# qq456cvb/CanonicalVoting

Hardware: AMD Instinct MI355X
Metric: scenes/sec (80k-pt synthetic scans) (higher is better)
Workload: dtype f32

## Files before the change

### canonicalvoting_amd/_lib.py

```python
import ctypes
import os
import threading

_HERE = os.path.dirname(os.path.abspath(__file__))
LIB_PATH = os.path.join(_HERE, "_C", "libcvhip.so")

c_float_p = ctypes.POINTER(ctypes.c_float)
c_int_p = ctypes.POINTER(ctypes.c_int)
c_i32_p = ctypes.POINTER(ctypes.c_int32)
c_i64_p = ctypes.POINTER(ctypes.c_int64)
vp = ctypes.c_void_p
ABI_VERSION = 6


class CvError(RuntimeError):
    pass


class DecodeParams(ctypes.Structure):
    _fields_ = [("thresh_high", ctypes.c_float), ("thresh_low", ctypes.c_float),
                ("valid_ratio", ctypes.c_float), ("elimination", ctypes.c_int),
                ("prob_thresh", ctypes.c_float), ("elim_hi_plus1", ctypes.c_int),
                ("max_iters", ctypes.c_int), ("err_thresh", ctypes.c_double)]

# ... 116 lines not shown
                ("d_points", vp), ("points_ld", ctypes.c_longlong), ("d_rgb", vp), ("d_owner", vp),
                ("d_minv", vp), ("d_model_scale", vp), ("d_model_cls", vp), ("n_models", ctypes.c_int),
                ("d_colour", vp), ("d_jitter", vp), ("n_clouds", ctypes.c_int),
                ("use_xyz", ctypes.c_int), ("recentre", ctypes.c_int),
                ("d_feats", vp), ("feats_ld", ctypes.c_longlong), ("d_xyz", vp), ("xyz_ld", ctypes.c_longlong),
                ("d_scale", vp), ("scale_ld", ctypes.c_longlong), ("d_cls", vp), ("cls_ld", ctypes.c_longlong)]


class SymLossDesc(ctypes.Structure):
    _fields_ = [("d_out", vp), ("n_rows", ctypes.c_longlong), ("ld", ctypes.c_longlong),
                ("d_rows", vp), ("d_pseg", vp), ("n_points", ctypes.c_longlong),
                ("d_seg_ptr", vp), ("d_pose_ptr", vp), ("d_tgt_ptr", vp), ("n_segments", ctypes.c_int), ("n_jobs", ctypes.c_int),
                ("d_targets", vp), ("n_targets", ctypes.c_longlong),
                ("d_urow", vp), ("d_uptr", vp), ("d_upoint", vp), ("n_urows", ctypes.c_int),
                ("w", ctypes.c_float * 3), ("xyz_factor", ctypes.c_float),
                ("d_loss", vp), ("d_pose_loss", vp), ("d_best", vp), ("d_seg_loss", vp),
                ("d_grad_loss", vp), ("d_grad", vp), ("grad_ld", ctypes.c_longlong),
                ("d_ws", vp), ("ws_bytes", ctypes.c_size_t)]


class SymRowsDesc(ctypes.Structure):
    _fields_ = [("d_coords4", vp), ("d_index", vp), ("d_inverse", vp), ("d_quant_counts", vp), ("m_points", ctypes.c_longlong),
                ("d_points", vp), ("points_ld", ctypes.c_longlong), ("d_rgb", vp), ("d_owner", vp),
                ("d_model_scale", vp), ("d_model_cls", vp), ("n_models", ctypes.c_int),
                ("d_colour", vp), ("d_jitter", vp), ("d_offsets", vp), ("n_clouds", ctypes.c_int),
                ("d_seg_vertex", vp), ("n_cand", ctypes.c_longlong),
                ("d_seg_vptr", vp), ("d_seg_pose_ptr", vp), ("n_seg_in", ctypes.c_int),
                ("d_minv", vp), ("n_jobs_in", ctypes.c_longlong), ("n_targets_in", ctypes.c_longlong),
                ("reference_indexing", ctypes.c_int), ("use_xyz", ctypes.c_int), ("recentre", ctypes.c_int),
                ("d_rows", vp), ("d_pseg", vp), ("d_seg_ptr", vp), ("d_pose_ptr", vp), ("d_tgt_ptr", vp), ("d_targets", vp),
                ("d_urow", vp), ("d_uptr", vp), ("d_upoint", vp),
                ("d_feats", vp), ("feats_ld", ctypes.c_longlong), ("d_scale", vp), ("scale_ld", ctypes.c_longlong),
                ("d_obj", vp), ("d_cls", vp), ("d_counts", vp), ("h_counts", vp),
                ("d_ws", vp), ("ws_bytes", ctypes.c_size_t)]


SYM_ROWS_COUNTS = ("P", "S", "J", "T", "U", "max_row", "N", "rejected")


class PointsFront(ctypes.Structure):
    _fields_ = [("d_raw_points", vp), ("m", ctypes.c_longlong), ("points_ld", ctypes.c_longlong), ("points_f64", ctypes.c_int),
                ("quantization_size", ctypes.c_double), ("d_raw_feats", vp), ("raw_feats_ld", ctypes.c_longlong),
                ("in_channels", ctypes.c_int), ("recentre_from", ctypes.c_int), ("d_raw_xyz", vp), ("d_raw_scale", vp),
                ("d_raw_prob", vp), ("d_raw_class", vp), ("d_coords4", vp), ("d_index", vp), ("d_inverse", vp)]


class PointsDesc(ctypes.Structure):
    _fields_ = [("front", PointsFront), ("scene", SceneDesc)]


class PointsSeparateDesc(ctypes.Structure):
    _fields_ = [("front", PointsFront), ("scene", SceneSeparateDesc)]


class PointsResult(ctypes.Structure):
    _fields_ = [("scene", SceneResult), ("n", ctypes.c_longlong), ("rejected", ctypes.c_int), ("host_us_front", ctypes.c_float),
                ("front_ws_bytes", ctypes.c_size_t), ("d_feats", vp), ("d_points", vp), ("d_xyz_in", vp), ("d_scale_in", vp),
                ("d_prob_in", vp), ("d_class_in", vp)]


class PointsSeparateResult(ctypes.Structure):
    _fields_ = [("scene", SceneSeparateResult), ("n", ctypes.c_longlong), ("rejected", ctypes.c_int),
                ("host_us_front", ctypes.c_float), ("front_ws_bytes", ctypes.c_size_t), ("d_feats", vp), ("d_points", vp),
                ("d_xyz_in", vp), ("d_scale_in", vp), ("d_prob_in", vp)]


SIGNATURES = {
    "cv_abi_version": (ctypes.c_int, []),
    "cv_last_error": (ctypes.c_char_p, []),
    "cv_hv_minmax_workspace_bytes": (ctypes.c_size_t, []),
    "cv_hv_minmax_f32": (ctypes.c_int, [vp, ctypes.c_int64, c_float_p, c_float_p, vp, ctypes.c_size_t, vp]),
    "cv_hv_minmax_async_f32": (ctypes.c_int, [vp, ctypes.c_int64, vp, vp, ctypes.c_size_t, vp]),
    "cv_hv_grid_dims_f32": (ctypes.c_int, [c_float_p, c_float_p, ctypes.c_float, c_int_p]),
    "cv_hv_forward_workspace_bytes": (ctypes.c_size_t, [ctypes.c_int64, ctypes.c_int, c_int_p, ctypes.c_int]),
    "cv_hv_forward_f32": (ctypes.c_int, [vp, vp, vp, vp, ctypes.c_int64, ctypes.c_float, ctypes.c_int,
                                         c_float_p, c_int_p, vp, vp, vp, vp, ctypes.c_size_t,
                                         ctypes.c_int, vp]),
    "cv_hv_forward_cat_workspace_bytes": (ctypes.c_size_t, [ctypes.c_int64, ctypes.c_int, c_int_p, ctypes.c_int, ctypes.c_int]),
    "cv_hv_forward_cat_f32": (ctypes.c_int, [vp, vp, vp, vp, ctypes.c_int64, ctypes.c_float, ctypes.c_int, c_float_p, c_int_p,
                                             ctypes.c_int, vp, vp, vp, vp, ctypes.c_size_t, ctypes.c_int, vp]),
    "cv_hv_forward_peaks_f32": (ctypes.c_int, [vp, vp, vp, vp, ctypes.c_int64, ctypes.c_float, ctypes.c_int,
                                               c_float_p, c_int_p, vp, vp, vp, vp, ctypes.c_size_t,
                                               ctypes.c_int, ctypes.c_float, vp]),
    "cv_hv_forward_peaks_cat_f32": (ctypes.c_int, [vp, vp, vp, vp, ctypes.c_int64, ctypes.c_float, ctypes.c_int, c_float_p, c_int_p,
                                                   ctypes.c_int, vp, vp, vp, vp, ctypes.c_size_t, ctypes.c_int, ctypes.c_float,
                                                   vp]),
    "cv_hv_set_kernel_events": (ctypes.c_int, [vp, vp]),
    "cv_hv_backward_f32": (ctypes.c_int, [vp, vp, vp, vp, vp, ctypes.c_int64, ctypes.c_float,
                                          ctypes.c_int, c_float_p, c_int_p, vp, vp, vp, vp]),
    "cv_hv_count_votes_f32": (ctypes.c_int, [vp, vp, vp, ctypes.c_int64, ctypes.c_float, ctypes.c_int,
                                             c_float_p, c_int_p, c_i64_p, vp, ctypes.c_size_t, vp]),
    "cv_decode_workspace_bytes": (ctypes.c_size_t, [c_int_p, ctypes.c_int64, ctypes.c_int]),
    "cv_decode_f32": (ctypes.c_int, [vp, vp, vp, c_int_p, c_float_p, ctypes.c_float, vp, vp, vp, vp,
                                     ctypes.c_int64, ctypes.POINTER(DecodeParams), ctypes.c_int, vp,
                                     ctypes.c_size_t, c_int_p, c_i64_p, c_i32_p, c_int_p, c_float_p,
                                     c_float_p, c_i32_p, c_int_p, vp]),
    "cv_decode_cat_workspace_bytes": (ctypes.c_size_t, [c_int_p, ctypes.c_int64, ctypes.c_int, ctypes.c_int]),
    "cv_decode_cat_f32": (ctypes.c_int, [vp, vp, vp, c_int_p, c_float_p, ctypes.c_float, vp, vp, vp, vp, ctypes.c_int64,
                                         ctypes.c_int, ctypes.POINTER(DecodeParams), ctypes.c_int, vp, ctypes.c_size_t, c_int_p,
                                         c_i64_p, c_i32_p, c_int_p, c_float_p, c_float_p, c_i32_p, c_int_p, vp]),
    "cv_detect_scene_separate_f32": (ctypes.c_int, [ctypes.POINTER(SceneSeparateDesc), ctypes.POINTER(SceneSeparateResult), vp]),
    "cv_sp_table_capacity": (ctypes.c_longlong, [ctypes.c_longlong]),
    "cv_sp_levels_workspace_bytes": (ctypes.c_size_t, [ctypes.c_longlong]),
    "cv_sp_build_levels": (ctypes.c_int, [ctypes.POINTER(vp), ctypes.POINTER(vp), ctypes.POINTER(vp),
                                          ctypes.c_longlong, ctypes.c_longlong, ctypes.c_int, vp,
                                          c_i32_p, vp, ctypes.c_size_t, vp]),
    "cv_sp_quantize_workspace_bytes": (ctypes.c_size_t, [ctypes.c_longlong]),
    "cv_sp_quantize_f32": (ctypes.c_int, [vp, ctypes.c_longlong, ctypes.c_longlong, ctypes.c_float, ctypes.c_int, c_i64_p,
                                          ctypes.c_int, vp, vp, vp, vp, c_i32_p, vp, ctypes.c_size_t, vp]),
    "cv_sp_quantize_f64": (ctypes.c_int, [vp, ctypes.c_longlong, ctypes.c_longlong, ctypes.c_double, ctypes.c_int, c_i64_p,
                                          ctypes.c_int, vp, vp, vp, vp, c_i32_p, vp, ctypes.c_size_t, vp]),
    "cv_sp_voxel_rows_f32": (ctypes.c_int, [vp, vp, ctypes.c_longlong, ctypes.c_float, vp, ctypes.POINTER(GatherJob), ctypes.c_int, vp]),
    "cv_sizeof_gather_job": (ctypes.c_size_t, []),
    "cv_sp_scan_rows_f32": (ctypes.c_int, [ctypes.POINTER(ScanRowsDesc), vp]),
    "cv_sizeof_scan_rows_desc": (ctypes.c_size_t, []),
    "cv_sym_loss_fwd_f32": (ctypes.c_int, [ctypes.POINTER(SymLossDesc), vp]),
    "cv_sym_loss_bwd_f32": (ctypes.c_int, [ctypes.POINTER(SymLossDesc), vp]),
    "cv_sym_loss_workspace_bytes": (ctypes.c_size_t, [ctypes.c_longlong, ctypes.c_int]),
    "cv_sym_loss_chunk_rows": (ctypes.c_int, []),
    "cv_sizeof_sym_loss_desc": (ctypes.c_size_t, []),
    "cv_sp_sym_rows_f32": (ctypes.c_int, [ctypes.POINTER(SymRowsDesc), vp]),
    "cv_sp_sym_rows_workspace_bytes": (ctypes.c_size_t, [ctypes.c_longlong, ctypes.c_longlong, ctypes.c_int, ctypes.c_int]),
    "cv_sp_sym_rows_block": (ctypes.c_int, []),
    "cv_sp_sym_rows_scan_span": (ctypes.c_longlong, []),
    "cv_sizeof_sym_rows_desc": (ctypes.c_size_t, []),
    "cv_sp_morton_keys": (ctypes.c_int, [vp, ctypes.c_longlong, vp, vp]),
    "cv_sp_sort_workspace_bytes": (ctypes.c_size_t, [ctypes.c_longlong]),
    "cv_sp_sort_rows": (ctypes.c_int, [vp, ctypes.c_longlong, vp, vp, vp, vp, ctypes.c_size_t, vp]),
    "cv_sp_pack_weights_stem_h2_f32": (ctypes.c_int, [vp, ctypes.c_int, ctypes.c_int, vp, ctypes.c_int, vp, vp]),
    "cv_sp_to_hl_f32": (ctypes.c_int, [vp, ctypes.c_longlong, ctypes.c_int, ctypes.c_int, vp, ctypes.c_int, vp, vp]),
    "cv_sp_from_hl_f32": (ctypes.c_int, [vp, ctypes.c_longlong, ctypes.c_int, ctypes.c_int, vp, ctypes.c_int, vp]),
    "cv_sp_kernel_map": (ctypes.c_int, [vp, ctypes.c_longlong, vp, vp, ctypes.c_longlong, ctypes.c_int,
                                        ctypes.c_int, vp, vp]),
    "cv_sp_up_map": (ctypes.c_int, [vp, ctypes.c_longlong, ctypes.c_longlong, vp, vp]),
    "cv_sp_conv_workspace_bytes": (ctypes.c_size_t, [ctypes.c_longlong, ctypes.c_int, ctypes.c_int]),
    "cv_sp_conv_f32": (ctypes.c_int, [ctypes.POINTER(ConvDesc), vp]),
    "cv_sp_set_split_target": (ctypes.c_int, [ctypes.c_int]),
    "cv_hv_set_part_records": (ctypes.c_int, [ctypes.c_int]),
    "cv_hv_set_part_records_thread": (ctypes.c_int, [ctypes.c_int]),
    "cv_sp_pack_weights_h2_batch_f32": (ctypes.c_int, [ctypes.POINTER(PackJob), ctypes.c_int, vp, vp]),
    "cv_sp_copy_unless_flag": (ctypes.c_int, [ctypes.POINTER(vp), ctypes.POINTER(vp), ctypes.POINTER(ctypes.c_longlong), ctypes.c_int, vp, vp]),
    "cv_sp_pack_weights_t_f32": (ctypes.c_int, [vp, ctypes.c_int, ctypes.c_int, ctypes.c_int, ctypes.c_int, ctypes.c_int, vp, vp]),
    "cv_sp_set_split_target_thread": (ctypes.c_int, [ctypes.c_int]),
    "cv_sp_set_ablation": (ctypes.c_int, [ctypes.c_int]),
    "cv_sp_set_option": (ctypes.c_int, [ctypes.c_char_p, ctypes.c_longlong, ctypes.POINTER(ctypes.c_longlong)]),
    "cv_sp_get_option": (ctypes.c_int, [ctypes.c_char_p, ctypes.POINTER(ctypes.c_longlong)]),
    "cv_sp_pack_weights_x6_f32": (ctypes.c_int, [vp, ctypes.c_int, ctypes.c_int, ctypes.c_int, vp, vp, vp]),
    "cv_sp_pack_weights_h2_f32": (ctypes.c_int, [vp, ctypes.c_int, ctypes.c_int, ctypes.c_int, vp, ctypes.c_int, vp, vp]),
    "cv_sp_pack_weights_bf16_f32": (ctypes.c_int, [vp, ctypes.c_int, ctypes.c_int, ctypes.c_int, vp, vp, vp]),
    "cv_sp_scene_maps_words": (ctypes.c_size_t, [c_i64_p, ctypes.c_longlong, ctypes.c_int, ctypes.c_int,
                                                 ctypes.c_longlong, ctypes.POINTER(SceneMaps)]),
    "cv_sp_scene_maps": (ctypes.c_int, [ctypes.POINTER(vp), ctypes.POINTER(vp), ctypes.POINTER(vp), ctypes.c_longlong,
                                        c_i64_p, vp, ctypes.c_longlong, ctypes.c_int,
                                        ctypes.c_int, ctypes.c_longlong, vp, ctypes.c_size_t, vp]),
    "cv_sp_scene_plan_words": (ctypes.c_size_t, [ctypes.c_longlong, ctypes.c_int, ctypes.c_int, ctypes.c_longlong]),
    "cv_sp_scene_plan": (ctypes.c_int, [vp, ctypes.c_longlong, vp, vp, ctypes.POINTER(vp), ctypes.POINTER(vp),
                                        ctypes.POINTER(vp), ctypes.c_longlong, vp, c_i32_p, ctypes.c_int, ctypes.c_int,
                                        ctypes.c_longlong, vp, ctypes.c_size_t, ctypes.POINTER(SceneMaps), vp,
                                        ctypes.c_size_t, vp, ctypes.c_size_t, vp]),
    "cv_sp_scene_plan_layout": (ctypes.c_int, [ctypes.c_longlong, ctypes.c_int, ctypes.c_int, ctypes.c_longlong,
                                               ctypes.POINTER(ScenePlanLayout)]),
    "cv_sp_scene_plan_slots": (ctypes.c_int, [ctypes.POINTER(ScenePlanLayout), ctypes.POINTER(SceneMaps), c_i64_p,
                                              ctypes.c_longlong, vp, ctypes.POINTER(vp), ctypes.POINTER(vp)]),
    "cv_sp_scene_conv_workspace_bytes": (ctypes.c_size_t, [c_i64_p, c_int_p, ctypes.c_int, ctypes.c_int]),
    "cv_net_arena_bytes": (ctypes.c_size_t, [ctypes.POINTER(NetBuf), ctypes.c_int, c_i64_p, ctypes.c_int]),
    "cv_net_run_f32": (ctypes.c_int, [ctypes.POINTER(NetOp), ctypes.c_int, ctypes.POINTER(NetBuf), ctypes.c_int,
# ... 111 lines not shown
```

### canonicalvoting_amd/csrc/cv_common.h

```cpp
#pragma once
#include <hip/hip_runtime.h>

#include <cstdarg>
#include <cstdint>
#include <cstdio>

#include "cv_hip.h"

void cv_set_error(const char* fmt, ...);

#define CV_HIP_CHECK(expr)                                                                  \
    do {                                                                                    \
        hipError_t e_ = (expr);                                                             \
        if (e_ != hipSuccess) {                                                             \
            cv_set_error("%s failed: %s (%s:%d)", #expr, hipGetErrorString(e_), __FILE__,   \
                         __LINE__);                                                         \
            return CV_EHIP;                                                                 \
        }                                                                                   \
    } while (0)

#define CV_LAUNCH_CHECK() CV_HIP_CHECK(hipGetLastError())

#define CV_REQUIRE(cond, code, ...)     \
    do {                                \
        if (!(cond)) {                  \
            cv_set_error(__VA_ARGS__);  \
            return (code);              \
        }                               \
    } while (0)

__host__ __device__ static inline size_t cv_align_up(size_t v, size_t a) { return (v + a - 1) / a * a; }

struct CvCarver {
    char* base;
    size_t off = 0;
    explicit CvCarver(void* p) : base(static_cast<char*>(p)) {}
    template <typename T>
    T* take(size_t count) {
        off = cv_align_up(off, 256);
        T* r = reinterpret_cast<T*>(base + off);
        off += count * sizeof(T);
        return r;
    }
};

struct CvMapJob {
    const int32_t* out_coords; long long n_out;
    const unsigned long long* keys; const int32_t* vals; long long cap;
    int k, ts;
    int32_t* nbr;
    const int32_t* compose;
    const unsigned* bitmap;
    const int32_t* bbox;
    int up;
    int32_t* nbr3;
    int32_t* mask_words;
};
constexpr int CV_MAX_MAP_JOBS = 12;
int cv_sp_kernel_maps_batch(const CvMapJob* jobs, int n_jobs, void* stream);
constexpr long long CV_BITMAP_WORDS = 1ll << 20;

int cv_sp_build_levels_zero(int32_t* const* d_coords, unsigned long long* const* d_keys, int32_t* const* d_vals,
                            long long n, long long cap, int num_levels, int32_t* d_counts, int32_t* h_counts, void* d_ws,
                            size_t ws_bytes, int32_t* d_zero, long long n_zero, int32_t* d_bbox, uint32_t* d_bits,
                            void* stream);

struct CvPermJob {
    const int32_t* nbr; long long n; int K, groups; int32_t* perm; int with_map;
    const int32_t* mask_words;
};
constexpr int CV_MAX_PERM_JOBS = 8;
int cv_hv_minmax_async_ex(const float* d_points, int64_t n, float* h_minmax6, void* d_ws, size_t ws_bytes, int32_t* d_zero_word,
                          int32_t* d_fill7f, void* stream);
struct DecodeCall {
    float* d_grid_obj; const float* d_grid_rot; const float* d_grid_scale;
    const int* dims; const float* h_corner3; float res;
    const float* d_points; const float* d_xyz; const float* d_prob; const int32_t* d_class; int64_t n;
    const cv_decode_params* params; int mutate_grid;
    void* d_ws; size_t ws_bytes;
    int* h_n_cand; int64_t* h_cand_idx; int32_t* h_verdict; int* h_n_boxes; float* h_boxes; float* h_scores; int32_t* h_classes;
    int* h_truncated;
    void* stream; void* ev_done;
};
int cv_decode_run(const DecodeCall& c, int num_cats, bool need_class);
int cv_sp_sort_rows_ex(const int32_t* d_coords, long long n, int32_t* d_sorted, int32_t* d_perm, int32_t* d_inv, void* d_ws,
                       size_t ws_bytes, bool single_batch, void* stream, bool bounds_prefilled);
int cv_sp_scene_plan_ex(const int32_t* d_input, long long n, int32_t* d_perm, int32_t* d_inv, int32_t* const* d_coords,
                        unsigned long long* const* d_keys, int32_t* const* d_vals, long long cap, int32_t* d_counts,
                        int32_t* h_counts, int stem_k, int mask_groups, long long masked_min_rows,
                        int32_t* d_arena, size_t arena_words, cv_scene_maps* offsets, void* d_sort_ws, size_t sort_ws_bytes,
                        void* d_levels_ws, size_t levels_ws_bytes, bool single_batch, void* stream,
                        bool bounds_prefilled);
int cv_sp_mask_perms_batch(const CvPermJob* jobs, int n_jobs, void* d_ws, size_t ws_bytes, void* stream,
                           bool pre_zeroed);

struct CvConvModels {
    int models;
    const cv_net_model_params* d_params;
    long long in_stride, in2_stride, res_stride, out_stride, ws_stride;
    int out_ext;
    float* ext_out[CV_MAX_CATEGORIES];
};
int cv_sp_conv_models_f32(const cv_conv_desc* d, const CvConvModels* mm, void* stream);
```

### canonicalvoting_amd/csrc/hv_decode.hip

```cpp
#include "cv_common.h"

#include <cmath>
#include <cstring>
#include <mutex>
#include <vector>

namespace {

constexpr int NCLS = 64;

struct Cand {
    long long idx;
    int c[3];
    int clo[3], chi[3];
    float cw[3];
    float cs, sn;
    float sc[3];
};

struct Stats {
    unsigned n_in, n_mask, pmax_bits;
    double err;
    unsigned hist[NCLS];
};
static_assert(offsetof(Stats, err) % 8 == 0, "64-bit atomic adds");
static_assert(sizeof(Stats) % 4 == 0, "a candidate's statistics are zeroed word by word");

struct Geo {
    int X, Y, Z;
    float corner[3];
    float res;
};

struct List {
    float* val;
    unsigned* xy;
    int* z;
    float* geo;
    int64_t cap;
};

__device__ __forceinline__ int cell_id(const Geo& geo, unsigned xy, int z) {
    return ((int)(xy & 0xffffu) * geo.Y + (int)(xy >> 16)) * geo.Z + z;
}

constexpr int CTR_WORDS = 16;
constexpr int CTR_LIST_N = 0;
constexpr int CTR_N_CAND = 4;

struct Ws {
    List L;
    unsigned* counters;
    Cand* cands;
    Stats* stats;
    __host__ __device__ unsigned* list_n() const { return counters + CTR_LIST_N; }
    __host__ __device__ int* n_cand() const { return reinterpret_cast<int*>(counters + CTR_N_CAND); }
};

struct CatStride { int64_t ws, n, cells; };
template <class T>
__device__ __forceinline__ void cat_shift(T*& p, int64_t bytes) {
    p = (T*)((char*)p + bytes);
}
__device__ __forceinline__ Ws cat(Ws w, int64_t stride, int k) {
    const int64_t o = (int64_t)k * stride;
    cat_shift(w.L.val, o); cat_shift(w.L.xy, o); cat_shift(w.L.z, o); cat_shift(w.L.geo, o);
    cat_shift(w.counters, o); cat_shift(w.cands, o); cat_shift(w.stats, o);
    return w;
}

__device__ __forceinline__ void lds_barrier() {
    asm volatile("s_waitcnt lgkmcnt(0)\n\ts_barrier" ::: "memory");
}

__device__ __forceinline__ int lanes_below(uint64_t mask) {
    return __builtin_amdgcn_mbcnt_hi((uint32_t)(mask >> 32),
                                     __builtin_amdgcn_mbcnt_lo((uint32_t)mask, 0));
}

__global__ __launch_bounds__(256) void dec_compact(const float* __restrict__ g_obj,
                                                   const float* __restrict__ g_rot,
                                                   const float* __restrict__ g_scale, Geo geo,
                                                   int64_t G, float thresh, Ws w, CatStride ks) {
    const int kc = blockIdx.y;
    g_obj = g_obj + kc * ks.cells; g_rot = g_rot + kc * 2 * ks.cells; g_scale = g_scale + kc * 3 * ks.cells;
    w = cat(w, ks.ws, kc);
    const List& L = w.L;
    unsigned* list_n = w.list_n();
    for (int64_t base = blockIdx.x * 256ll; base < G; base += (int64_t)gridDim.x * 256) {
        const int64_t i = base + threadIdx.x;
        float v = 0.f;
        bool hit = false;
        if (i < G) { v = g_obj[i]; hit = v >= thresh; }
        const uint64_t m = __ballot(hit);
        if (m == 0) continue;
        unsigned pos = 0;
        const int lane = threadIdx.x & 63;
        const int leader = __ffsll((unsigned long long)m) - 1;
        if (lane == leader) pos = atomicAdd(list_n, (unsigned)__popcll(m));
        pos = __shfl(pos, leader);
        if (hit) {
            const unsigned p = pos + lanes_below(m);
            const int id = (int)i;
            L.val[p] = v;
            const int z = id % geo.Z, y = (id / geo.Z) % geo.Y, x = id / (geo.Z * geo.Y);
            L.xy[p] = (unsigned)x | ((unsigned)y << 16);
            L.z[p] = z;
            const float r0 = g_rot[(int64_t)id * 2], r1 = g_rot[(int64_t)id * 2 + 1];
            const float rot = (float)atan2((double)r1, (double)r0);
            L.geo[0 * L.cap + p] = (float)cos((double)rot);
            L.geo[1 * L.cap + p] = (float)sin((double)rot);
            for (int k = 0; k < 3; ++k) L.geo[(2 + k) * L.cap + p] = g_scale[(int64_t)id * 3 + k];
        }
    }
}

__device__ __forceinline__ bool inv_coords(float d0, float d1, float d2, float c, float s,
                                           const float* sc, float& w0, float& w1, float& w2) {
    w0 = fmaf(d2, s, fmaf(d1, 0.f, d0 * c)) / sc[0];
    w1 = fmaf(d2, 0.f, fmaf(d1, 1.f, d0 * 0.f)) / sc[1];
    w2 = fmaf(d2, c, fmaf(d1, 0.f, d0 * (-s))) / sc[2];
    return -1 < w0 && w0 < 1 && -1 < w1 && w1 < 1 && -1 < w2 && w2 < 1;
}

__device__ __forceinline__ bool inside_box(float d0, float d1, float d2, float c, float s, const float* sc) {
    const float t0 = fmaf(d2, s, fmaf(d1, 0.f, d0 * c));
    const float t1 = fmaf(d2, 0.f, fmaf(d1, 1.f, d0 * 0.f));
    const float t2 = fmaf(d2, c, fmaf(d1, 0.f, d0 * (-s)));
    return fabsf(t0) < fabsf(sc[0]) && fabsf(t1) < fabsf(sc[1]) && fabsf(t2) < fabsf(sc[2]);
}

__device__ __forceinline__ void box_corners(float cs, float sn, const float* sc, float* bb) {
    constexpr float kRawX[8] = {1, 1, -1, -1, 1, 1, -1, -1};
    constexpr float kRawY[8] = {1, 1, 1, 1, -1, -1, -1, -1};
    constexpr float kRawZ[8] = {1, -1, -1, 1, 1, -1, -1, 1};
    const float m00 = cs * sc[0], m02 = (-sn) * sc[2], m11 = sc[1], m20 = sn * sc[0], m22 = cs * sc[2];
#pragma unroll
    for (int q = 0; q < 8; ++q) {
        bb[q * 3 + 0] = m00 * kRawX[q] + m02 * kRawZ[q];
        bb[q * 3 + 1] = m11 * kRawY[q];
        bb[q * 3 + 2] = m20 * kRawX[q] + m22 * kRawZ[q];
    }
}

struct Best {
    float v;
    int id, pos;
    int q;
};

__device__ __forceinline__ void take_better(Best& b, float v, int id, int pos, int q) {
    if (v > b.v || (v == b.v && id < b.id)) { b.v = v; b.id = id; b.pos = pos; b.q = q; }
}

constexpr int GREEDY_T = 512;
constexpr int GREEDY_CAP = 4096;

template <int CTRL>
__device__ __forceinline__ int dpp_mov(int x) {
    return __builtin_amdgcn_update_dpp(x, x, CTRL, 0xf, 0xf, false);
}
__device__ __forceinline__ float wave_max_f32(float x) {
    x = fmaxf(x, __int_as_float(dpp_mov<0xB1>(__float_as_int(x))));
    x = fmaxf(x, __int_as_float(dpp_mov<0x4E>(__float_as_int(x))));
    x = fmaxf(x, __int_as_float(dpp_mov<0x124>(__float_as_int(x))));
    x = fmaxf(x, __int_as_float(dpp_mov<0x128>(__float_as_int(x))));
    const int xi = __float_as_int(x);
    const float a = __int_as_float(__builtin_amdgcn_readlane(xi, 0)), b = __int_as_float(__builtin_amdgcn_readlane(xi, 16)),
                c = __int_as_float(__builtin_amdgcn_readlane(xi, 32)), d = __int_as_float(__builtin_amdgcn_readlane(xi, 48));
    return fmaxf(fmaxf(a, b), fmaxf(c, d));
}
__device__ __forceinline__ int wave_min_i32(int x) {
    x = min(x, dpp_mov<0xB1>(x));
    x = min(x, dpp_mov<0x4E>(x));
    x = min(x, dpp_mov<0x124>(x));
    x = min(x, dpp_mov<0x128>(x));
    return min(min(__builtin_amdgcn_readlane(x, 0), __builtin_amdgcn_readlane(x, 16)),
               min(__builtin_amdgcn_readlane(x, 32), __builtin_amdgcn_readlane(x, 48)));
}

template <int W, class Also>
__device__ __forceinline__ Best best_of_workgroup(float (&s_val)[2][W], int (&s_idx)[2][W], int (&s_pos)[2][W], int it, float bv,
                                                  int bid, int bpos, Also&& also) {
    const int wave = threadIdx.x >> 6, par = it & 1;
    const float wv = wave_max_f32(bv);
    const int wid = wave_min_i32(bv == wv ? bid : 0x7fffffff);
    if (bv == wv && bid == wid) {
        s_val[par][wave] = bv; s_idx[par][wave] = bid; s_pos[par][wave] = bpos;
        also(par, wave);
    }
    lds_barrier();
    Best w{s_val[par][0], s_idx[par][0], s_pos[par][0], 0};
#pragma unroll
    for (int q = 1; q < W; ++q) take_better(w, s_val[par][q], s_idx[par][q], s_pos[par][q], q);
    return w;
// ... 472 lines not shown
    const int nx = cd.chi[0] - cd.clo[0] + 1, ny = cd.chi[1] - cd.clo[1] + 1,
              nz = cd.chi[2] - cd.clo[2] + 1;
    for (int64_t t = threadIdx.x; t < (int64_t)nx * ny * nz; t += 256) {
        const int z = cd.clo[2] + (int)(t % nz), y = cd.clo[1] + (int)((t / nz) % ny),
                  x = cd.clo[0] + (int)(t / ((int64_t)nz * ny));
        float w0, w1, w2;
        if (inv_coords((float)(x - cd.c[0]) * geo.res, (float)(y - cd.c[1]) * geo.res,
                       (float)(z - cd.c[2]) * geo.res, cd.cs, cd.sn, cd.sc, w0, w1, w2))
            g_obj[((int64_t)x * geo.Y + y) * geo.Z + z] = 0.f;
    }
}

__global__ __launch_bounds__(64) void dec_zero_counters(Ws w, int64_t ks_ws) {
    w = cat(w, ks_ws, blockIdx.y);
    if (threadIdx.x < CTR_WORDS) w.counters[threadIdx.x] = 0u;
}

struct WsLayout {
    size_t off_val, off_xy, off_z, off_geo, off_counters, off_cands, off_stats, total;
    int64_t cells;
    WsLayout(int64_t G, int M) : cells(G) {
        size_t o = 0;
        off_val = o; o = cv_align_up(o + sizeof(float) * G, 256);
        off_xy = o; o = cv_align_up(o + sizeof(unsigned) * G, 256);
        off_z = o; o = cv_align_up(o + sizeof(int) * G, 256);
        off_geo = o; o = cv_align_up(o + sizeof(float) * 5 * G, 256);
        off_counters = o; o = cv_align_up(o + sizeof(unsigned) * CTR_WORDS, 256);
        off_cands = o; o = cv_align_up(o + sizeof(Cand) * M, 256);
        off_stats = o; o = cv_align_up(o + sizeof(Stats) * M, 256);
        o = cv_align_up(o + ResultLayout(M).total, 256);
        total = o;
    }
    Ws at(char* ws) const {
        Ws w;
        w.L.val = reinterpret_cast<float*>(ws + off_val);
        w.L.xy = reinterpret_cast<unsigned*>(ws + off_xy);
        w.L.z = reinterpret_cast<int*>(ws + off_z);
        w.L.geo = reinterpret_cast<float*>(ws + off_geo);
        w.L.cap = cells;
        w.counters = reinterpret_cast<unsigned*>(ws + off_counters);
        w.cands = reinterpret_cast<Cand*>(ws + off_cands);
        w.stats = reinterpret_cast<Stats*>(ws + off_stats);
        return w;
    }
};

struct PinnedPool {
    std::mutex mu;
    std::vector<std::pair<char*, size_t>> free_list;
    std::pair<char*, size_t> take(size_t bytes) {
        {
            std::lock_guard<std::mutex> g(mu);
            for (size_t i = 0; i < free_list.size(); ++i)
                if (free_list[i].second >= bytes) {
                    const std::pair<char*, size_t> b = free_list[i];
                    free_list.erase(free_list.begin() + i);
                    return b;
                }
        }
        void* p = nullptr;
        if (hipHostMalloc(&p, bytes, hipHostMallocMapped) != hipSuccess) return {nullptr, 0};
        return {static_cast<char*>(p), bytes};
    }
    void give(std::pair<char*, size_t> b) {
        std::lock_guard<std::mutex> g(mu);
        if (free_list.size() < 64) free_list.push_back(b);
        else (void)hipHostFree(b.first);
    }
};
PinnedPool g_pinned;

struct PinnedLease {
    const std::pair<char*, size_t> buf;
    explicit PinnedLease(size_t bytes) : buf(g_pinned.take(bytes)) {}
    ~PinnedLease() { if (buf.first) g_pinned.give(buf); }
    PinnedLease(const PinnedLease&) = delete;
    PinnedLease& operator=(const PinnedLease&) = delete;
};

}

int cv_decode_run(const DecodeCall& c, int K, bool need_class) {
    CV_REQUIRE(K >= 1 && K <= CV_MAX_CATEGORIES, CV_EINVAL, "num_cats out of range (%d, 1..%d)", K, CV_MAX_CATEGORIES);
    CV_REQUIRE(c.d_grid_obj && c.d_grid_rot && c.d_grid_scale && c.dims && c.h_corner3 && c.d_points && c.d_xyz && c.d_prob &&
                   (c.d_class || !need_class) && c.params && c.d_ws && c.h_n_cand && c.h_cand_idx && c.h_verdict && c.h_n_boxes &&
                   c.h_boxes && c.h_scores && c.h_classes,
               CV_EINVAL, "null pointer argument");
    const int* dims = c.dims;
    const cv_decode_params* params = c.params;
    const int64_t n = c.n;
    hipStream_t st = static_cast<hipStream_t>(c.stream);
    CV_REQUIRE(n > 0, CV_EINVAL, "n must be positive");
    CV_REQUIRE(c.res > 0.f, CV_EINVAL, "res must be positive");
    CV_REQUIRE(dims[0] > 0 && dims[1] > 0 && dims[2] > 0, CV_EINVAL, "bad grid dims");
    CV_REQUIRE(dims[0] < 65536 && dims[1] < 65536 && dims[2] < 65536, CV_EINVAL, "grid dims must be below 65536");
    const int64_t G = (int64_t)dims[0] * dims[1] * dims[2];
    CV_REQUIRE(G < (1ll << 31), CV_EINVAL, "grid too large");
    const int M = params->max_iters;
    CV_REQUIRE(M > 0 && M <= 65536, CV_EINVAL, "max_iters out of range");
    CV_REQUIRE(params->elimination >= 0, CV_EINVAL, "elimination must be >= 0");
    CV_REQUIRE(params->thresh_high > 0.f, CV_EINVAL, "thresh_high must be positive");
    const WsLayout W(G, M);
    const size_t need = (size_t)K * W.total;
    CV_REQUIRE(c.ws_bytes >= need, CV_ENOMEM, "workspace too small (%zu < %zu)", c.ws_bytes, need);
    const Ws w = W.at(static_cast<char*>(c.d_ws));
    const ResultLayout RL(M);
    const PinnedLease lease((size_t)K * RL.total);
    char* host = lease.buf.first;
    CV_REQUIRE(host != nullptr, CV_ENOMEM, "pinned host buffer of %zu bytes", (size_t)K * RL.total);
    const CatStride ks{K > 1 ? (int64_t)W.total : 0, n, G};

    if (K == 1) CV_HIP_CHECK(hipMemsetAsync(w.counters, 0, sizeof(unsigned) * CTR_WORDS, st));
    else {
        dec_zero_counters<<<dim3(1, K), 64, 0, st>>>(w, ks.ws);
        CV_LAUNCH_CHECK();
    }
    Geo geo{dims[0], dims[1], dims[2], {c.h_corner3[0], c.h_corner3[1], c.h_corner3[2]}, c.res};
    const int cblocks = (int)std::min<int64_t>((G + 255) / 256, 2048);
    dec_compact<<<dim3(cblocks, K), 256, 0, st>>>(c.d_grid_obj, c.d_grid_rot, c.d_grid_scale, geo, G, params->thresh_high, w, ks);
    CV_LAUNCH_CHECK();
    static const long long big_cells = getenv("CV_DEC_BIG_CELLS") ? atoll(getenv("CV_DEC_BIG_CELLS")) : (4ll << 20);
    if (G > big_cells) dec_greedy_dispatch_big<<<dim3(1, K), GREEDY_T_BIG, 0, st>>>(geo, *params, w, ks.ws);
    else dec_greedy_dispatch<<<dim3(1, K), GREEDY_T, 0, st>>>(geo, *params, w, ks.ws);
    CV_LAUNCH_CHECK();
    const dim3 bgrid((unsigned)((n + 255) / 256), (unsigned)std::min((M + 7) / 8, 8), (unsigned)K);
    dec_backproject<<<bgrid, 256, 0, st>>>(c.d_points, c.d_xyz, c.d_prob, c.d_class, n, params->prob_thresh, w, ks);
    CV_LAUNCH_CHECK();
    dec_finalize<<<dim3(1, K), 256, 0, st>>>(w, *params, host, M, ks.ws, (int64_t)RL.total);
    CV_LAUNCH_CHECK();
    if (c.mutate_grid) {
        dec_apply<<<dim3(M, K), 256, 0, st>>>(c.d_grid_obj, geo, *params, w, ks);
        CV_LAUNCH_CHECK();
    }
    if (c.ev_done) CV_HIP_CHECK(hipEventRecord(static_cast<hipEvent_t>(c.ev_done), st));
    CV_HIP_CHECK(hipStreamSynchronize(st));
    for (int k = 0; k < K; ++k) {
        const char* hk = host + (size_t)k * RL.total;
        const int* hdr = reinterpret_cast<const int*>(hk);
        const int nc = hdr[0], nb = hdr[1];
        CV_REQUIRE(nc >= 0 && nc <= M && nb >= 0 && nb <= nc, CV_ERANGE, "corrupt decode result");
        c.h_n_cand[k] = nc;
        c.h_n_boxes[k] = nb;
        if (c.h_truncated) c.h_truncated[k] = hdr[2];
        std::memcpy(c.h_cand_idx + (size_t)k * M, hk + RL.off_cand, sizeof(int64_t) * nc);
        std::memcpy(c.h_verdict + (size_t)k * M, hk + RL.off_verdict, sizeof(int32_t) * nc);
        std::memcpy(c.h_boxes + (size_t)k * M * 24, hk + RL.off_boxes, sizeof(float) * 24 * nb);
        std::memcpy(c.h_scores + (size_t)k * M, hk + RL.off_scores, sizeof(float) * nb);
        std::memcpy(c.h_classes + (size_t)k * M, hk + RL.off_classes, sizeof(int32_t) * nb);
    }
    return CV_OK;
}

extern "C" {

size_t cv_decode_workspace_bytes(const int dims[3], int64_t n, int max_iters) {
    if (!dims || max_iters <= 0) return 0;
    (void)n;
    return WsLayout((int64_t)dims[0] * dims[1] * dims[2], max_iters).total;
}

size_t cv_decode_cat_workspace_bytes(const int dims[3], int64_t n, int max_iters, int num_cats) {
    if (num_cats < 1 || num_cats > CV_MAX_CATEGORIES) return 0;
    return (size_t)num_cats * cv_decode_workspace_bytes(dims, n, max_iters);
}

int cv_decode_f32(float* d_grid_obj, const float* d_grid_rot, const float* d_grid_scale,
                  const int dims[3], const float h_corner3[3], float res, const float* d_points,
                  const float* d_xyz, const float* d_prob, const int32_t* d_class, int64_t n,
                  const cv_decode_params* params, int mutate_grid, void* d_ws, size_t ws_bytes,
                  int* h_n_cand, int64_t* h_cand_idx, int32_t* h_verdict, int* h_n_boxes,
                  float* h_boxes, float* h_scores, int32_t* h_classes, int* h_truncated, void* stream) {
    const DecodeCall c{d_grid_obj, d_grid_rot, d_grid_scale, dims, h_corner3, res, d_points, d_xyz, d_prob, d_class, n, params,
                       mutate_grid, d_ws, ws_bytes, h_n_cand, h_cand_idx, h_verdict, h_n_boxes, h_boxes, h_scores, h_classes,
                       h_truncated, stream, nullptr};
    return cv_decode_run(c, 1, true);
}

int cv_decode_cat_f32(float* d_grid_obj, const float* d_grid_rot, const float* d_grid_scale, const int dims[3],
                      const float h_corner3[3], float res, const float* d_points, const float* d_xyz, const float* d_prob,
                      const int32_t* d_class, int64_t n, int num_cats, const cv_decode_params* params, int mutate_grid, void* d_ws,
                      size_t ws_bytes, int* h_n_cand, int64_t* h_cand_idx, int32_t* h_verdict, int* h_n_boxes, float* h_boxes,
                      float* h_scores, int32_t* h_classes, int* h_truncated, void* stream) {
    const DecodeCall c{d_grid_obj, d_grid_rot, d_grid_scale, dims, h_corner3, res, d_points, d_xyz, d_prob, d_class, n, params,
                       mutate_grid, d_ws, ws_bytes, h_n_cand, h_cand_idx, h_verdict, h_n_boxes, h_boxes, h_scores, h_classes,
                       h_truncated, stream, nullptr};
    return cv_decode_run(c, num_cats, false);
}

}
```

### canonicalvoting_amd/csrc/hv_vote.hip

```cpp
#include "cv_common.h"

#include <atomic>
#include <algorithm>
#include <cmath>
#include <cstddef>
#include <mutex>
#include <type_traits>
#include <unordered_map>
#include <vector>

namespace {

struct F3 { float x, y, z; };
struct I3 { int x, y, z; };

std::mutex g_tab_mu;
std::unordered_map<uint64_t, float2*> g_tabs;

int get_rot_table(int num_rots, const float2** out) {
    int dev = 0;
    CV_HIP_CHECK(hipGetDevice(&dev));
    const uint64_t key = (uint64_t(uint32_t(dev)) << 32) | uint32_t(num_rots);
    std::lock_guard<std::mutex> lk(g_tab_mu);
    auto it = g_tabs.find(key);
// ... 132 lines not shown

constexpr int TX = 16, TZ = 32, TCELLS = TX * TZ;
constexpr int TW = 8;
constexpr int LQ = TW * 64;
constexpr int CULL_BATCH = 4;
static_assert(CULL_BATCH >= 1 && CULL_BATCH <= 8, "one carry bit and one record index per sub-chunk and lane");
constexpr int VQ = 128;
constexpr int MAX_R_TILES = 256;
static_assert(MAX_R_TILES <= TW * 64, "the rotation table is staged by one load per lane");
constexpr int LIST_CHUNK = 16;
static_assert(64 % LIST_CHUNK == 0, "a wave takes 64 / LIST_CHUNK list chunks per hand-out, one entry per lane");
static_assert(LQ <= 512, "the list entry of a queued vote has 9 bits");
static_assert(MAX_R_TILES <= 256, "the rotation of a queued vote has 8 bits");
static_assert(TX + 1 < 64 && TZ + 1 < 64, "lx + 1 and lz + 1 of a queued vote have 6 bits each");
static_assert(TZ == 32, "acc_idx splits a cell index by >> 5 and & 31");

constexpr int LIST_CHUNK_RECORDS = 1024;
constexpr int PREP_MAX_Y = 4096;
constexpr int PREP_THREADS = 1024;

struct CatStride { int64_t ws, n, cells; };
template <class T>
__device__ __forceinline__ T* cat_ws(T* p, int64_t bytes) {
    return (T*)((const char*)p + (int64_t)blockIdx.y * bytes);
}
template <class T>
__device__ __forceinline__ T* cat_el(T* p, int64_t elems) {
    return p + (int64_t)blockIdx.y * elems;
}

__global__ __launch_bounds__(PREP_THREADS) void hv_prep_count(
    const float* __restrict__ pts, const float* __restrict__ xyz, const float* __restrict__ scl,
    int64_t n, float res, float corner_y, int Y, int* __restrict__ fy_out, int* __restrict__ ycount, CatStride ks) {
    __shared__ int lh[PREP_MAX_Y];
    xyz = cat_el(xyz, 3 * ks.n); scl = cat_el(scl, 3 * ks.n);
    fy_out = cat_ws(fy_out, ks.ws); ycount = cat_ws(ycount, ks.ws);
    const bool use_lds = Y <= PREP_MAX_Y;
    if (use_lds) {
        for (int i = threadIdx.x; i < Y; i += PREP_THREADS) lh[i] = 0;
        __syncthreads();
    }
    const int64_t c = blockIdx.x * (int64_t)PREP_THREADS + threadIdx.x;
    if (c < n) {
        const float cy = xyz[c * 3 + 1] * scl[c * 3 + 1];
        const float gy = grid_pos(pts[c * 3 + 1], -cy, corner_y, res);
        int fy = -1;
        if (gy >= 0 && gy < (float)(Y - 1)) fy = (int)gy;
        fy_out[c] = fy;
        if (fy >= 0) atomicAdd(use_lds ? &lh[fy] : &ycount[fy], 1);
    }
    if (use_lds) {
        __syncthreads();
        for (int i = threadIdx.x; i < Y; i += PREP_THREADS)
            if (lh[i]) atomicAdd(&ycount[i], lh[i]);
    }
}

constexpr int PART_RECORDS = 4096;
constexpr int MAX_PARTS = 8;

template <class V, class E>
__device__ __forceinline__ int wave_excl_scan(int Y, V value, E emit) {
    const int lane = threadIdx.x & 63;
    int carry = 0;
    for (int base = 0; base < Y; base += 64) {
        const int i = base + lane;
        const int v = i < Y ? value(i) : 0;
        int incl = v;
#pragma unroll
        for (int off = 1; off < 64; off <<= 1) {
            const int t = __shfl_up(incl, off);
            if (lane >= off) incl += t;
        }
        if (i < Y) emit(i, carry + incl - v, v);
        carry += __shfl(incl, 63);
    }
    return carry;
}
__global__ __launch_bounds__(256) void hv_prep_scan(const int* __restrict__ ycount, int Y,
                                                    int* __restrict__ ystart,
                                                    int* __restrict__ cursor,
                                                    int* __restrict__ part_start, int4* __restrict__ q_info, int max_q,
                                                    int* __restrict__ chunk_start, int* __restrict__ bin_of_chunk,
                                                    int part_records, int64_t ks_ws) {
    ycount = cat_ws(ycount, ks_ws); ystart = cat_ws(ystart, ks_ws); cursor = cat_ws(cursor, ks_ws);
    part_start = cat_ws(part_start, ks_ws); q_info = cat_ws(q_info, ks_ws);
    chunk_start = cat_ws(chunk_start, ks_ws); bin_of_chunk = cat_ws(bin_of_chunk, ks_ws);
    const int wave = threadIdx.x >> 6, lane = threadIdx.x & 63;
    if (wave == 0) {
        const int total = wave_excl_scan(Y, [&](int i) { return ycount[i]; },
                                         [&](int i, int excl, int) { ystart[i] = excl; cursor[i] = excl; });
        if (lane == 0) ystart[Y] = total;
    } else if (wave == 1) {
        const int total = wave_excl_scan(Y,
            [&](int i) {
                const int n2 = (i >= 1 ? ycount[i - 1] : 0) + (i <= Y - 2 ? ycount[i] : 0);
                return min(max((n2 + part_records - 1) / part_records, 1), MAX_PARTS);
            },
            [&](int i, int excl, int v) {
                part_start[i] = excl;
                for (int p2 = 0; p2 < v; ++p2) q_info[excl + p2] = make_int4(i, p2, v, excl);
            });
        for (int q = total + lane; q < max_q; q += 64) q_info[q] = make_int4(0, 0, -1, 0);
        if (lane == 0) part_start[Y] = total;
    } else if (wave == 2) {
        const int total = wave_excl_scan(Y, [&](int i) { return (ycount[i] + LIST_CHUNK_RECORDS - 1) / LIST_CHUNK_RECORDS; },
                                         [&](int i, int excl, int v) {
                                             chunk_start[i] = excl;
                                             for (int p2 = 0; p2 < v; ++p2) bin_of_chunk[excl + p2] = i;
                                         });
        if (lane == 0) chunk_start[Y] = total;
    }
}

constexpr int REC_F = 13;

__global__ __launch_bounds__(PREP_THREADS) void hv_prep_scatter(
    const float* __restrict__ pts, const float* __restrict__ xyz, const float* __restrict__ scl,
    const float* __restrict__ obj, const int* __restrict__ fy_in, int64_t n, int Y, float res,
    F3 corner, int* __restrict__ cursor, float* __restrict__ rec, int64_t rec_stride, CatStride ks) {
    __shared__ int lh[PREP_MAX_Y];
    xyz = cat_el(xyz, 3 * ks.n); scl = cat_el(scl, 3 * ks.n); obj = cat_el(obj, ks.n);
    fy_in = cat_ws(fy_in, ks.ws); cursor = cat_ws(cursor, ks.ws); rec = cat_ws(rec, ks.ws);
    const bool use_lds = Y <= PREP_MAX_Y;
    const int64_t c = blockIdx.x * (int64_t)PREP_THREADS + threadIdx.x;
    const int fy = c < n ? fy_in[c] : -1;
    int pos = -1;
    if (!use_lds) {
        if (fy >= 0) pos = atomicAdd(&cursor[fy], 1);
    } else {
        for (int i = threadIdx.x; i < Y; i += PREP_THREADS) lh[i] = 0;
        __syncthreads();
        int rank = 0;
        if (fy >= 0) rank = atomicAdd(&lh[fy], 1);
        __syncthreads();
        for (int i = threadIdx.x; i < Y; i += PREP_THREADS)
            if (lh[i]) lh[i] = atomicAdd(&cursor[i], lh[i]);
        __syncthreads();
        if (fy >= 0) pos = lh[fy] + rank;
    }
    if (pos < 0) return;
    const float px = pts[c * 3 + 0], py = pts[c * 3 + 1], pz = pts[c * 3 + 2];
    const float s0 = scl[c * 3 + 0], s1 = scl[c * 3 + 1], s2 = scl[c * 3 + 2];
    const float cx = xyz[c * 3 + 0] * s0, cy = xyz[c * 3 + 1] * s1, cz = xyz[c * 3 + 2] * s2;
    const float gy = grid_pos(py, -cy, corner.y, res);
    float* r = rec + pos;
    r[0 * rec_stride] = px;
    r[1 * rec_stride] = pz;
    r[2 * rec_stride] = cx;
    r[3 * rec_stride] = cz;
    r[4 * rec_stride] = gy - floorf(gy);
    r[5 * rec_stride] = obj[c];
    r[6 * rec_stride] = s0;
    r[7 * rec_stride] = s1;
    r[8 * rec_stride] = s2;
    r[9 * rec_stride] = (px - corner.x) / res;
    r[10 * rec_stride] = (pz - corner.z) / res;
    r[11 * rec_stride] = sqrtf(cx * cx + cz * cz) / res;
    r[12 * rec_stride] = atan2f(cz, cx) + 3.14159265f;
}


constexpr int LIST_MAX_TILES = 4096;
struct RingArc { bool keep; int a_start, a_len; };
__device__ __forceinline__ bool ring_touches(float ux, float uz, float r, float xlo, float xhi, float zlo, float zhi,
                                             float& dxn, float& dzn) {
    const float slack = 0.05f;
    dxn = fmaxf(0.f, fmaxf(xlo - ux, ux - xhi));
    dzn = fmaxf(0.f, fmaxf(zlo - uz, uz - zhi));
    const float dxf = fmaxf(fabsf(ux - xlo), fabsf(ux - xhi));
    const float dzf = fmaxf(fabsf(uz - zlo), fabsf(uz - zhi));
    const float dmin = sqrtf(dxn * dxn + dzn * dzn), dmax = sqrtf(dxf * dxf + dzf * dzf);
    const float tol = slack + 1e-5f * (r + fabsf(ux) + fabsf(uz));
    return (r >= dmin - tol) && (r <= dmax + tol);
}
__device__ __forceinline__ void ring_arc(float ux, float uz, float a0, int R, float xlo, float xhi, float zlo, float zhi,
                                         float dxn, float dzn, int& a_start, int& a_len) {
    a_start = 0;
    a_len = R;
    if (dxn + dzn > 0.5f) {
        const float b0 = atan2f(0.5f * (zlo + zhi) - uz, 0.5f * (xlo + xhi) - ux);
        float lo = 0.f, hi = 0.f;
#pragma unroll
        for (int k = 0; k < 4; ++k) {
            float d = atan2f(((k & 2) ? zhi : zlo) - uz, ((k & 1) ? xhi : xlo) - ux) - b0;
            d -= 6.28318531f * rintf(d * 0.159154943f);
            lo = fminf(lo, d);
            hi = fmaxf(hi, d);
        }
        const float inv_step = (float)R * 0.159154943f;
        float first = (b0 + lo - a0) * inv_step - 2.f;
        const int len = (int)((hi - lo) * inv_step) + 6;
        first -= (float)R * floorf(first / (float)R);
        a_start = min(max((int)first, 0), R - 1);
// ... 228 lines not shown
        rx = sh.vq_rx[wave][slot]; rz = sh.vq_rz[wave][slot];
        const int e = rec & 511, rot = (rec >> 9) & 255;
        lx = (int)((rec >> 17) & 63) - 1; lz = (int)((rec >> 23) & 63) - 1;
        wy = sh.pq[4][e]; ob = sh.pq[5][e];
        if constexpr (MODE != VOTE_OBJ) {
            s0 = sh.pq[6][e]; s1 = sh.pq[7][e]; s2 = sh.pq[8][e];
            cs = sh.tab[rot];
        }
    }
    const bool small = fabsf(ob) * fmaxf(1.f, fmaxf(fabsf(s0), fmaxf(fabsf(s1), fabsf(s2)))) < 16384.f;
    if (__all(small)) {
        if (active) drain_vote<true, MODE>(sh, lx, lz, rx, rz, wy, ob, s0, s1, s2, cs, box);
    } else {
        if (active) drain_vote<false, MODE>(sh, lx, lz, rx, rz, wy, ob, s0, s1, s2, cs, box);
    }
}

__device__ __forceinline__ void wave_sync_lds() {
    __builtin_amdgcn_fence(__ATOMIC_RELEASE, "wavefront");
    __builtin_amdgcn_wave_barrier();
    __builtin_amdgcn_fence(__ATOMIC_ACQUIRE, "wavefront");
}

__device__ __forceinline__ float arc_atan2(float y, float x) {
    const float ax = fabsf(x), ay = fabsf(y);
    const float a = fminf(ax, ay) * __builtin_amdgcn_rcpf(fmaxf(fmaxf(ax, ay), 1e-30f));
    const float q = a * a;
    float r = ((-0.0464964749f * q + 0.15931422f) * q - 0.327622764f) * q * a + a;
    r = ay > ax ? 1.57079637f - r : r;
    r = x < 0.f ? 3.14159274f - r : r;
    return y < 0.f ? -r : r;
}

__device__ __forceinline__ void edge_arc(float ux, float uz, float r, float a0, int R, float xlo, float xhi, float zlo,
                                         float zhi, int& a_start, int& a_len) {
    if (!(r >= 2.f)) return;
    const float slack = 0.05f, half_pi = 1.57079637f, two_pi = 6.28318531f;
    const float d4[4] = {xhi - ux, zhi - uz, ux - xlo, uz - zlo};
    const float inv_r = 1.f / r;
    float h[4];
#pragma unroll
    for (int k = 0; k < 4; ++k) {
        const float t = (d4[k] + slack) * inv_r;
        const float hk = arc_atan2(sqrtf(fmaxf(1.f - t * t, 0.f)), t) - 0.01f;
        h[k] = (t < 1.f && hk > 0.f) ? hk : -1.f;
    }
    float best = 0.f, best_end = 0.f;
#pragma unroll
    for (int k = 0; k < 4; ++k) {
        float lo = -h[k], hi = h[k];
        bool ok = h[k] > 0.f;
        if (ok && hi - lo > best) { best = hi - lo; best_end = (float)k * half_pi + hi; }
#pragma unroll
        for (int j = 1; j < 4; ++j) {
            const float hp = h[(k + j - 1) & 3], hn = h[(k + j) & 3];
            ok = ok && hn > 0.f && hp + hn >= half_pi;
            if (ok) {
                lo = fminf(lo, (float)j * half_pi - hn);
                hi = fmaxf(hi, (float)j * half_pi + hn);
                if (hi - lo > best) { best = hi - lo; best_end = (float)k * half_pi + hi; }
            }
        }
    }
    const float inside = fmaxf(two_pi - best, 0.f);
    const float inv_step = (float)R * 0.159154943f;
    const int len = (int)(inside * inv_step) + 6;
    if (len < a_len) {
        float first = (best_end - a0) * inv_step - 2.f;
        first -= (float)R * floorf(first / (float)R);
        a_start = min(max((int)first, 0), R - 1);
        a_len = len;
    }
}

template <bool QUEUE, int MODE>
__device__ __forceinline__ void hv_tile_item(
    int y, int tile, int part, int nparts, int slot0, int slot_stride,
    int R, float res, F3 corner, I3 dims,
    const int* __restrict__ ystart, const float* __restrict__ rec,
    int64_t rec_stride, int tiles_x, int tiles_z, unsigned long long* __restrict__ partials,
    int* __restrict__ arrivals, float* __restrict__ g_obj, float* __restrict__ g_rot,
    float* __restrict__ g_scale, const int* __restrict__ list_ctl, const int* __restrict__ list_start, const int* __restrict__ list_cnt,
    const int2* __restrict__ entries, int list_mode ,
    int4* __restrict__ hot, float thresh, int4* __restrict__ hot_items, const float2* __restrict__ tab) {
    constexpr int NCH = vote_channels(MODE);
    __shared__ TileSharedT<MODE> sh;
    __shared__ int last_flag;
    __shared__ int hot_lds[MODE == VOTE_OBJ ? 4 : 1];
    const int X = dims.x, Y = dims.y, Z = dims.z;
    const int ntiles = tiles_x * tiles_z;
    const int x0 = (tile / tiles_z) * TX, z0 = (tile % tiles_z) * TZ;
    const int lane = threadIdx.x & 63, wave = threadIdx.x >> 6;
    HotBox box{0, TX - 1, 0, TZ - 1};
    if (MODE == VOTE_PEAKS) {
        const int4 h = hot[y * ntiles + tile];
        box = HotBox{h.x, h.y, h.z, h.w};
        if (box.x0 > box.x1) return;
    }
    if (nparts == 0) {
        const int nx0 = min(TX, X - x0), nz0 = min(TZ, Z - z0);
        for (int i = threadIdx.x; i < TCELLS; i += TW * 64) {
            const int lx = i / TZ, lz = i % TZ;
            if (lx < nx0 && lz < nz0) {
                const int64_t cell = ((int64_t)(x0 + lx) * Y + y) * Z + z0 + lz;
                if (MODE != VOTE_PEAKS) g_obj[cell] = 0.f;
                if (MODE != VOTE_OBJ) {
                    reinterpret_cast<float2*>(g_rot)[cell] = make_float2(0.f, 0.f);
                    g_scale[cell * 3 + 0] = 0.f; g_scale[cell * 3 + 1] = 0.f; g_scale[cell * 3 + 2] = 0.f;
                }
            }
        }
        if (MODE == VOTE_OBJ && threadIdx.x == 0) {
            hot[y * ntiles + tile] = 0.f >= thresh ? make_int4(0, nx0 - 1, 0, nz0 - 1) : make_int4(TX, -1, TZ, -1);
            if (0.f >= thresh) hot_items[atomicAdd(&arrivals[Y * ntiles], 1)] = make_int4(y, tile, 0, slot0);
        }
        return;
    }
    const bool use_list = QUEUE && list_mode == 2 && list_ctl[1] == 0;
    int lbeg[2] = {0, 0}, llen[2] = {0, 0};
    if (use_list) {
#pragma unroll
        for (int k = 0; k < 2; ++k) {
            const int s = y - 1 + k;
            if (s >= 0 && s <= Y - 2) {
                lbeg[k] = list_start[(int64_t)s * ntiles + tile];
                llen[k] = list_cnt[(int64_t)s * ntiles + tile];
            }
        }
    }

    int bin_beg[2], bin_end[2];
#pragma unroll
    for (int k = 0; k < 2; ++k) {
        const int s = y - 1 + k;
        const bool valid = s >= 0 && s <= Y - 2;
        bin_beg[k] = !valid ? 0 : (use_list ? lbeg[k] : ystart[s]);
        bin_end[k] = !valid ? 0 : (use_list ? lbeg[k] + llen[k] : ystart[s + 1]);
    }
    const float2 tab_mine = (int)threadIdx.x < R ? tab[threadIdx.x] : make_float2(0.f, 0.f);
    for (int i = threadIdx.x; i < TileSharedT<MODE>::ACC_WORDS; i += TW * 64) sh.acc[i] = 0ull;
    if ((int)threadIdx.x < R) sh.tab[threadIdx.x] = tab_mine;
    if (threadIdx.x < 2) sh.next_chunk[threadIdx.x] = 0;
    if (threadIdx.x == 2) { sh.list_len = 0; sh.more = 0; }
    if (MODE == VOTE_OBJ && threadIdx.x >= 4 && threadIdx.x < 8)
        hot_lds[threadIdx.x - 4] = (threadIdx.x & 1) ? -1 : (threadIdx.x == 4 ? TX : TZ);
    __syncthreads();

    const float slack = 0.05f;
    const float xlo = MODE == VOTE_PEAKS ? (float)(x0 + box.x0 - 1) : (float)(x0 - 1),
                xhi = MODE == VOTE_PEAKS ? (float)(x0 + box.x1 + 1) : (float)(x0 + TX),
                zlo = MODE == VOTE_PEAKS ? (float)(z0 + box.z0 - 1) : (float)(z0 - 1),
                zhi = MODE == VOTE_PEAKS ? (float)(z0 + box.z1 + 1) : (float)(z0 + TZ);
    int vq_len = 0;

    const int per = use_list ? LIST_CHUNK : 64;
    int sb = 0;
    int c_mask = 0, c_idx[CULL_BATCH], c_arc = 0, c_k = 0;
#pragma unroll
    for (int j = 0; j < CULL_BATCH; ++j) c_idx[j] = 0;
    auto append = [&](int mask, const int (&idx)[CULL_BATCH], int arc, int k) -> int {
        int tot = 0, before[CULL_BATCH];
#pragma unroll
        for (int j = 0; j < CULL_BATCH; ++j) {
            const uint64_t m = __ballot((mask >> j) & 1);
            before[j] = tot + lanes_below(m);
            tot += __popcll(m);
        }
        if (tot == 0) return 0;
        int p0 = 0;
        if (lane == 0) p0 = atomicAdd(&sh.list_len, tot);
        p0 = __builtin_amdgcn_readfirstlane(p0);
#pragma unroll
        for (int j = 0; j < CULL_BATCH; ++j) {
            const int pos = p0 + before[j];
            if (((mask >> j) & 1) && pos < LQ) {
                sh.arc_start[pos] = idx[j] | (int)((unsigned)k << 31);
                if (use_list) sh.arc_cum[pos] = arc;
                mask &= ~(1 << j);
            }
        }
        return mask;
    };

    for (;;) {
        bool more = false;
        if (__ballot(c_mask != 0) != 0) {
            c_mask = append(c_mask, c_idx, c_arc, c_k);
            more = __ballot(c_mask != 0) != 0;
        }
// ... 151 lines not shown
            float rx = 0, rz = 0;
            if (it0 < it1) {
                if (it0 == e_end) {
                    ++e;
                    e_end = sh.arc_cum[e];
                    rot = sh.arc_start[e];
                    epx = sh.pq[0][e]; epz = sh.pq[1][e];
                    ecx = sh.pq[2][e]; ecz = sh.pq[3][e];
                }
                const float2 cs = sh.tab[rot];
                const float ox = (-cs.x) * ecx + cs.y * ecz;
                const float oz = (-cs.y) * ecx - cs.x * ecz;
                const float gx = grid_pos(epx, ox, corner.x, res);
                const float gz = grid_pos(epz, oz, corner.z, res);
                if (gx >= 0 && gz >= 0 && gx < (float)(X - 1) && gz < (float)(Z - 1)) {
                    const int lx = (int)gx - x0, lz = (int)gz - z0;
                    if (MODE == VOTE_PEAKS ? (lx >= box.x0 - 1 && lx <= box.x1 && lz >= box.z0 - 1 && lz <= box.z1)
                                           : (lx >= -1 && lx < TX && lz >= -1 && lz < TZ)) {
                        isvote = true;
                        rx = gx - floorf(gx);
                        rz = gz - floorf(gz);
                        vrec = (uint32_t)e | ((uint32_t)rot << 9) | ((uint32_t)(lx + 1) << 17) |
                               ((uint32_t)(lz + 1) << 23);
                    }
                }
                if (++rot == R) rot = 0;
            }
            const uint64_t mv = __ballot(isvote);
            if (isvote) {
                const int q = vq_len + lanes_below(mv);
                sh.vq_rec[wave][q] = vrec;
                sh.vq_rx[wave][q] = rx;
                sh.vq_rz[wave][q] = rz;
            }
            vq_len += __popcll(mv);
            wave_sync_lds();
            if (vq_len >= 64) {
                vq_len -= 64;
                drain64<MODE>(sh, wave, vq_len + lane, true, box);
            }
        }
        if (vq_len > 0) {
            drain64<MODE>(sh, wave, lane, lane < vq_len, box);
            vq_len = 0;
        }
        wave_sync_lds();
        if (!again) break;
        __syncthreads();
    }
    __syncthreads();

    if (nparts > 1) {
        unsigned long long* mine = partials + ((int64_t)slot0 + (int64_t)part * slot_stride) * (6 * TCELLS);
        for (int i = threadIdx.x; i < NCH * TCELLS; i += TW * 64) mine[i] = sh.acc[acc_idx(i / TCELLS, i % TCELLS)];
        asm volatile("s_waitcnt vmcnt(0)" ::: "memory");
        __syncthreads();
        if (threadIdx.x == 0) {
            __builtin_amdgcn_fence(__ATOMIC_RELEASE, "agent");
            asm volatile("s_waitcnt vmcnt(0)" ::: "memory");
            const int old = __hip_atomic_fetch_add(&arrivals[y * ntiles + tile], 1, __ATOMIC_RELAXED,
                                                   __HIP_MEMORY_SCOPE_AGENT);
            last_flag = old == nparts - 1;
            if (last_flag) __builtin_amdgcn_fence(__ATOMIC_ACQUIRE, "agent");
            if (MODE == VOTE_OBJ && last_flag)
                __hip_atomic_store(&arrivals[y * ntiles + tile], 0, __ATOMIC_RELAXED, __HIP_MEMORY_SCOPE_AGENT);
        }
        __syncthreads();
        if (!last_flag) return;
        const unsigned long long* base = partials + (int64_t)slot0 * (6 * TCELLS);
        for (int i = threadIdx.x; i < NCH * TCELLS; i += TW * 64) {
            unsigned long long sum = 0ull;
            for (int p2 = 0; p2 < nparts; ++p2) sum += base[(int64_t)p2 * slot_stride * (6 * TCELLS) + i];
            sh.acc[acc_idx(i / TCELLS, i % TCELLS)] = sum;
        }
        __syncthreads();
    }

    const int nx = min(TX, X - x0), nz = min(TZ, Z - z0);
    if constexpr (MODE == VOTE_OBJ) {
        for (int i = threadIdx.x; i < TCELLS; i += TW * 64) {
            const int lx = i / TZ, lz = i % TZ;
            if (lx < nx && lz < nz) {
                const float v = (float)fx_value(sh.acc[acc_idx(0, i)]);
                g_obj[((int64_t)(x0 + lx) * Y + y) * Z + z0 + lz] = v;
                if (v >= thresh) {
                    atomicMin(&hot_lds[0], lx); atomicMax(&hot_lds[1], lx);
                    atomicMin(&hot_lds[2], lz); atomicMax(&hot_lds[3], lz);
                }
            }
        }
        __syncthreads();
        if (threadIdx.x == 0) {
            hot[y * ntiles + tile] = make_int4(hot_lds[0], hot_lds[1], hot_lds[2], hot_lds[3]);
            if (hot_lds[0] <= hot_lds[1]) {
                const int at = atomicAdd(&arrivals[Y * ntiles], nparts);
                for (int p2 = 0; p2 < nparts; ++p2) hot_items[at + p2] = make_int4(y, tile, p2 | (nparts << 8), slot0);
            }
        }
    } else if constexpr (MODE == VOTE_PEAKS) {
        for (int i = threadIdx.x; i < TCELLS; i += TW * 64) {
            const int lx = i / TZ, lz = i % TZ;
            if (lx < box.x0 || lx > box.x1 || lz < box.z0 || lz > box.z1) continue;
            const int64_t cell = ((int64_t)(x0 + lx) * Y + y) * Z + z0 + lz;
            const float v = g_obj[cell];
            if (!(v >= thresh)) continue;
            const double d = (double)v + 1e-7;
#pragma unroll
            for (int j = 0; j < 2; ++j) g_rot[cell * 2 + j] = (float)((double)(float)fx_value(sh.acc[acc_idx(j, i)]) / d);
#pragma unroll
            for (int j = 0; j < 3; ++j) g_scale[cell * 3 + j] = (float)((double)(float)fx_value(sh.acc[acc_idx(2 + j, i)]) / d);
        }
    } else {
        for (int i = threadIdx.x; i < TCELLS; i += TW * 64) {
            const int lx = i / TZ, lz = i % TZ;
            if (lx < nx && lz < nz)
                g_obj[((int64_t)(x0 + lx) * Y + y) * Z + z0 + lz] = (float)fx_value(sh.acc[acc_idx(0, i)]);
        }
        for (int i = threadIdx.x; i < TCELLS * 2; i += TW * 64) {
            const int cell = i >> 1, j = i & 1;
            const int lx = cell / TZ, lz = cell % TZ;
            if (lx < nx && lz < nz) {
                const double d = (double)(float)fx_value(sh.acc[acc_idx(0, cell)]) + 1e-7;
                g_rot[(((int64_t)(x0 + lx) * Y + y) * Z + z0 + lz) * 2 + j] =
                    (float)((double)(float)fx_value(sh.acc[acc_idx(1 + j, cell)]) / d);
            }
        }
        for (int i = threadIdx.x; i < TCELLS * 3; i += TW * 64) {
            const int cell = i / 3, j = i - cell * 3;
            const int lx = cell / TZ, lz = cell % TZ;
            if (lx < nx && lz < nz) {
                const double d = (double)(float)fx_value(sh.acc[acc_idx(0, cell)]) + 1e-7;
                g_scale[(((int64_t)(x0 + lx) * Y + y) * Z + z0 + lz) * 3 + j] =
                    (float)((double)(float)fx_value(sh.acc[acc_idx(3 + j, cell)]) / d);
            }
        }
    }
}

template <bool QUEUE, int MODE>
__global__ __launch_bounds__(TW * 64) void hv_fwd_tiles(
    int R, float res, F3 corner, I3 dims, const float2* __restrict__ tab,
    const int* __restrict__ ystart, const int4* __restrict__ items, const float* __restrict__ rec,
    int64_t rec_stride, int tiles_x, int tiles_z, unsigned long long* __restrict__ partials,
    int* __restrict__ arrivals, float* __restrict__ g_obj, float* __restrict__ g_rot,
    float* __restrict__ g_scale, const int* __restrict__ list_ctl, const int* __restrict__ list_start, const int* __restrict__ list_cnt,
    const int2* __restrict__ entries, int list_mode ,
    const int4* __restrict__ q_info, CatStride ks, int4* __restrict__ hot, float thresh, int4* __restrict__ hot_items) {
    ystart = cat_ws(ystart, ks.ws); items = cat_ws(items, ks.ws); rec = cat_ws(rec, ks.ws);
    partials = cat_ws(partials, ks.ws); arrivals = cat_ws(arrivals, ks.ws); list_ctl = cat_ws(list_ctl, ks.ws);
    list_start = cat_ws(list_start, ks.ws); list_cnt = cat_ws(list_cnt, ks.ws); entries = cat_ws(entries, ks.ws);
    q_info = cat_ws(q_info, ks.ws);
    g_obj = cat_el(g_obj, ks.cells); g_rot = cat_el(g_rot, 2 * ks.cells); g_scale = cat_el(g_scale, 3 * ks.cells);
    if (MODE != VOTE_FULL) { hot = cat_ws(hot, ks.ws); hot_items = cat_ws(hot_items, ks.ws); }
    const int ntiles = tiles_x * tiles_z;
#define CV_TILE_ITEM_ARGS R, res, corner, dims, ystart, rec, rec_stride, tiles_x, tiles_z, partials, arrivals, g_obj, g_rot, g_scale, \
                          list_ctl, list_start, list_cnt, entries, list_mode, hot, thresh, hot_items
    if (MODE == VOTE_PEAKS) {
        const int count = arrivals[dims.y * ntiles];
        if ((int)blockIdx.x >= count) return;
        for (int i = blockIdx.x; i < count; i += gridDim.x) {
            const int4 item = hot_items[i];
            hv_tile_item<QUEUE, MODE>(item.x, item.y, item.z & 0xff, item.z >> 8, item.w, QUEUE ? 1 : ntiles, CV_TILE_ITEM_ARGS, tab);
            __syncthreads();
        }
        return;
    }
    int y, tile, part, nparts, slot0, slot_stride;
    if (QUEUE) {
        if ((int)blockIdx.x >= list_ctl[2]) return;
        const int4 item = items[blockIdx.x];
        y = item.x; tile = item.y; part = item.z & 0xff; nparts = item.z >> 8; slot0 = item.w; slot_stride = 1;
    } else {
        tile = blockIdx.x % ntiles;
        const int4 qi = q_info[blockIdx.x / ntiles];
        if (qi.z < 0) return;
        y = qi.x; part = qi.y; nparts = qi.z;
        slot0 = qi.w * ntiles + tile; slot_stride = ntiles;
    }
    hv_tile_item<QUEUE, MODE>(y, tile, part, nparts, slot0, slot_stride, CV_TILE_ITEM_ARGS, tab);
#undef CV_TILE_ITEM_ARGS
}

__global__ __launch_bounds__(256) void hv_bwd(
    const float* __restrict__ grad, const float* __restrict__ pts, const float* __restrict__ xyz,
    const float* __restrict__ scl, const float* __restrict__ obj, int64_t n, int R, float res,
    F3 corner, I3 dims, const float2* __restrict__ tab, float* __restrict__ d_xyz,
    float* __restrict__ d_scl, float* __restrict__ d_obj) {
    const int lane = threadIdx.x & 63;
    const int64_t c = blockIdx.x * 4ll + (threadIdx.x >> 6);
    if (c >= n) return;
    const int Y = dims.y, Z = dims.z;
    const float s0 = scl[c * 3 + 0], s1 = scl[c * 3 + 1], s2 = scl[c * 3 + 2];
    const float x0 = xyz[c * 3 + 0], x1 = xyz[c * 3 + 1], x2 = xyz[c * 3 + 2];
    const float cx = x0 * s0, cy = x1 * s1, cz = x2 * s2;
    const float px = pts[c * 3 + 0], py = pts[c * 3 + 1], pz = pts[c * 3 + 2];
    const float ob = obj[c];
    float a_obj = 0, a_x0 = 0, a_x1 = 0, a_x2 = 0, a_s0 = 0, a_s1 = 0, a_s2 = 0;
    for (int i = lane; i < R; i += 64) {
        const float2 cs = tab[i];
        const float ox = (-cs.x) * cx + cs.y * cz;
        const float oy = -cy;
        const float oz = (-cs.y) * cx - cs.x * cz;
        const float gx = grid_pos(px, ox, corner.x, res);
        const float gy = grid_pos(py, oy, corner.y, res);
        const float gz = grid_pos(pz, oz, corner.z, res);
        if (gx < 0 || gy < 0 || gz < 0 || gx >= (float)(dims.x - 1) || gy >= (float)(dims.y - 1) ||
            gz >= (float)(dims.z - 1))
            continue;
        const int fx = (int)gx, fy = (int)gy, fz = (int)gz;
        const float rx = gx - floorf(gx), ry = gy - floorf(gy), rz = gz - floorf(gz);
        const float w0x = 1.f - rx, w0y = 1.f - ry, w0z = 1.f - rz, w1x = rx, w1y = ry, w1z = rz;
        const int64_t b = ((int64_t)fx * Y + fy) * Z + fz;
        const int64_t sx = (int64_t)Y * Z, sy = Z;
        const float lll = grad[b], llh = grad[b + 1], lhl = grad[b + sy], lhh = grad[b + sy + 1];
        const float hll = grad[b + sx], hlh = grad[b + sx + 1], hhl = grad[b + sx + sy],
                    hhh = grad[b + sx + sy + 1];
        float dob = lll * w0x * w0y * w0z;
        dob += llh * w0x * w0y * w1z;
        dob += lhl * w0x * w1y * w0z;
        dob += lhh * w0x * w1y * w1z;
        dob += hll * w1x * w0y * w0z;
        dob += hlh * w1x * w0y * w1z;
        dob += hhl * w1x * w1y * w0z;
        dob += hhh * w1x * w1y * w1z;
        a_obj += dob;
        float dx = -lll * w0y * w0z;
        dx = dx - llh * w0y * w1z; dx = dx - lhl * w1y * w0z; dx = dx - lhh * w1y * w1z;
        dx = dx + hll * w0y * w0z; dx = dx + hlh * w0y * w1z; dx = dx + hhl * w1y * w0z;
        dx = dx + hhh * w1y * w1z;
        float dy = -lll * w0x * w0z;
        dy = dy - llh * w0x * w1z; dy = dy + lhl * w0x * w0z; dy = dy + lhh * w0x * w1z;
        dy = dy - hll * w1x * w0z; dy = dy - hlh * w1x * w1z; dy = dy + hhl * w1x * w0z;
        dy = dy + hhh * w1x * w1z;
        float dz = -lll * w0x * w0y;
        dz = dz + llh * w0x * w0y; dz = dz - lhl * w0x * w1y; dz = dz + lhh * w0x * w1y;
        dz = dz - hll * w1x * w0y; dz = dz + hlh * w1x * w0y; dz = dz - hhl * w1x * w1y;
        dz = dz + hhh * w1x * w1y;
        dx *= ob; dy *= ob; dz *= ob;
        const float dcx = (-cs.x) * dx - cs.y * dz;
// ... 152 lines not shown
    const int rc = cv_hv_minmax_async_ex(d_points, n, h, d_ws, ws_bytes, nullptr, nullptr, stream);
    if (rc) return rc;
    CV_HIP_CHECK(hipStreamSynchronize(static_cast<hipStream_t>(stream)));
    for (int k = 0; k < 3; ++k) { h_min3[k] = h[k]; h_max3[k] = h[3 + k]; }
    return CV_OK;
}

int cv_hv_minmax_async_f32(const float* d_points, int64_t n, float* h_minmax6, void* d_ws, size_t ws_bytes,
                           void* stream) {
    return cv_hv_minmax_async_ex(d_points, n, h_minmax6, d_ws, ws_bytes, nullptr, nullptr, stream);
}

}

int cv_hv_minmax_async_ex(const float* d_points, int64_t n, float* h_minmax6, void* d_ws, size_t ws_bytes, int32_t* d_zero_word,
                          int32_t* d_fill7f, void* stream) {
    CV_REQUIRE(d_points && h_minmax6 && d_ws, CV_EINVAL, "null pointer argument");
    CV_REQUIRE(n > 0, CV_EINVAL, "n must be positive (got %lld)", (long long)n);
    CV_REQUIRE(ws_bytes >= cv_hv_minmax_workspace_bytes(), CV_ENOMEM, "workspace too small");
    hipStream_t st = static_cast<hipStream_t>(stream);
    CvCarver cv(d_ws);
    float* part = cv.take<float>(6 * MM_BLOCKS);
    float* out = cv.take<float>(6);
    const int blocks = (int)std::min<int64_t>(MM_BLOCKS, (n + 255) / 256);
    minmax_partial<<<blocks, 256, 0, st>>>(d_points, n, part);
    CV_LAUNCH_CHECK();
    minmax_final<<<1, 256, 0, st>>>(part, blocks, out, d_zero_word, d_fill7f);
    CV_LAUNCH_CHECK();
    CV_HIP_CHECK(hipMemcpyAsync(h_minmax6, out, 6 * sizeof(float), hipMemcpyDeviceToHost, st));
    return CV_OK;
}

extern "C" {

int cv_hv_grid_dims_f32(const float h_min3[3], const float h_max3[3], float res, int dims_out[3]) {
    CV_REQUIRE(h_min3 && h_max3 && dims_out, CV_EINVAL, "null pointer argument");
    CV_REQUIRE(res > 0.f, CV_EINVAL, "res must be positive");
    for (int k = 0; k < 3; ++k) {
        volatile float d = h_max3[k] - h_min3[k];
        volatile float q = d / res;
        dims_out[k] = (int)q + 1;
    }
    return CV_OK;
}

size_t cv_hv_forward_workspace_bytes(int64_t n, int num_rots, const int dims[3], int algo) {
    if (!dims || n <= 0 || !algo_ok(algo)) return 0;
    if (pick_algo(algo, n, num_rots) == 1) return 256;
    return tiles_layout(n, num_rots, dims, nullptr).bytes;
}

static thread_local hipEvent_t t_ev_start = nullptr, t_ev_stop = nullptr;

static std::atomic<long long> g_part_records{getenv("CV_HV_PART_RECORDS") ? std::max<long long>(PART_RECORDS, atoll(getenv("CV_HV_PART_RECORDS")))
                                                                          : (long long)PART_RECORDS};

static thread_local long long t_part_records = 0;

int cv_hv_set_part_records(int records) {
    const long long v = records <= 0 ? (long long)PART_RECORDS : std::max<long long>(PART_RECORDS, records);
    return (int)g_part_records.exchange(v, std::memory_order_relaxed);
}

int cv_hv_set_part_records_thread(int records) {
    const int before = (int)t_part_records;
    t_part_records = records <= 0 ? 0 : std::max<long long>(PART_RECORDS, records);
    return before;
}

int cv_hv_set_kernel_events(void* ev_start, void* ev_stop) {
    t_ev_start = static_cast<hipEvent_t>(ev_start);
    t_ev_stop = static_cast<hipEvent_t>(ev_stop);
    return CV_OK;
}

size_t cv_hv_forward_cat_workspace_bytes(int64_t n, int num_rots, const int dims[3], int algo, int num_cats) {
    if (num_cats < 1 || num_cats > CV_MAX_CATEGORIES) return 0;
    return (size_t)num_cats * cv_hv_forward_workspace_bytes(n, num_rots, dims, algo);
}

static int hv_forward_cats(const float* d_points, const float* d_xyz, const float* d_scale, const float* d_obj, int64_t n,
                           float res, int num_rots, const float h_corner3[3], const int dims[3], float* d_grid_obj,
                           float* d_grid_rot, float* d_grid_scale, void* d_ws, size_t ws_bytes, int algo, int K,
                           hipStream_t st, bool peaks = false, float thresh = 0.f) {
    int rc = CV_OK;
    const float2* tab = nullptr;
    rc = get_rot_table(num_rots, &tab);
    if (rc) return rc;
    const F3 corner{h_corner3[0], h_corner3[1], h_corner3[2]};
    const I3 d3{dims[0], dims[1], dims[2]};
    const int64_t cells = (int64_t)dims[0] * dims[1] * dims[2];
    const int a = pick_algo(algo, n, num_rots);
    if (a == 2) CV_REQUIRE(num_rots <= MAX_R_TILES, CV_EINVAL, "tiles algorithm needs num_rots <= %d", MAX_R_TILES);
    if (a == 1) {
        for (int k = 0; k < K; ++k) {
            float* g_obj = d_grid_obj + (int64_t)k * cells;
            float* g_rot = d_grid_rot + (int64_t)k * cells * 2;
            float* g_scale = d_grid_scale + (int64_t)k * cells * 3;
            CV_HIP_CHECK(hipMemsetAsync(g_obj, 0, sizeof(float) * cells, st));
            CV_HIP_CHECK(hipMemsetAsync(g_rot, 0, sizeof(float) * cells * 2, st));
            CV_HIP_CHECK(hipMemsetAsync(g_scale, 0, sizeof(float) * cells * 3, st));
            const int64_t total = n * num_rots;
            hv_fwd_direct<<<(unsigned)((total + 255) / 256), 256, 0, st>>>(
                d_points, d_xyz + (int64_t)k * n * 3, d_scale + (int64_t)k * n * 3, d_obj + (int64_t)k * n, n, num_rots, res,
                corner, d3, tab, g_obj, g_rot, g_scale);
            CV_LAUNCH_CHECK();
            hv_normalise<<<(unsigned)((cells + 255) / 256), 256, 0, st>>>(g_obj, g_rot, g_scale, cells);
            CV_LAUNCH_CHECK();
        }
        return CV_OK;
    }
    const int Y = dims[1];
    const TilesLayout L = tiles_layout(n, num_rots, dims, d_ws);
    CV_REQUIRE(d_ws && ws_bytes >= (size_t)K * L.bytes, CV_ENOMEM, "workspace too small for the tiles algorithm");
    const CatStride ks{K > 1 ? (int64_t)L.bytes : 0, n, cells};
    const int tiles_x = L.tiles_x, tiles_z = L.tiles_z, ntiles = L.ntiles;
    const bool queue = L.queue;
    const int list_mode = queue ? 2 : 1;
    if (K == 1) CV_HIP_CHECK(hipMemsetAsync(L.zero_from, 0, L.zero_bytes, st));
    else {
        hv_zero_cat<<<dim3((unsigned)std::min<size_t>((L.zero_bytes / 4 + 255) / 256, 1024), K), 256, 0, st>>>(L.zero_from,
                                                                                                          L.zero_bytes / 4, ks.ws);
        CV_LAUNCH_CHECK();
    }
    const unsigned prep_wgs = (unsigned)((n + PREP_THREADS - 1) / PREP_THREADS);
    hv_prep_count<<<dim3(prep_wgs, K), PREP_THREADS, 0, st>>>(d_points, d_xyz, d_scale, n, res, corner.y, Y, L.fy, L.ycount, ks);
    CV_LAUNCH_CHECK();
    hv_prep_scan<<<dim3(1, K), 256, 0, st>>>(L.ycount, Y, L.ystart, L.cursor, L.part_start, L.q_info, (int)L.max_q, L.chunk_start,
                                             L.bin_of_chunk,
                                             (int)(t_part_records > 0 ? t_part_records : g_part_records.load(std::memory_order_relaxed)),
                                             ks.ws);
    CV_LAUNCH_CHECK();
    hv_prep_scatter<<<dim3(prep_wgs, K), PREP_THREADS, 0, st>>>(d_points, d_xyz, d_scale, d_obj, L.fy, n, Y, res, corner, L.cursor,
                                                                 L.rec, n, ks);
    CV_LAUNCH_CHECK();
    if (queue) {
        hv_list_pass<false><<<dim3((unsigned)L.max_chunks, K), 1024, 0, st>>>(L.ystart, L.chunk_start, L.bin_of_chunk, Y, L.rec, n,
                                                                               num_rots, tiles_x, tiles_z, L.list_ctl, L.list_cnt,
                                                                               L.list_start, L.chunk_off, L.entries, L.tile_w, 1, ks.ws);
        CV_LAUNCH_CHECK();
        hv_build_queue<<<dim3(1, K), 1024, 0, st>>>(L.tile_w, Y, ntiles, (int)L.max_items, (int)L.max_slots, L.list_ctl, L.items,
                                                    ks.ws);
        CV_LAUNCH_CHECK();
        hv_list_scan<<<dim3(1, K), 1024, 0, st>>>(L.list_cnt, Y, ntiles, L.list_cap, L.list_ctl, L.list_start, ks.ws);
        CV_LAUNCH_CHECK();
        hv_list_pass<true><<<dim3((unsigned)L.max_chunks, K), 1024, 0, st>>>(L.ystart, L.chunk_start, L.bin_of_chunk, Y, L.rec, n,
                                                                              num_rots, tiles_x, tiles_z, L.list_ctl, L.list_cnt,
                                                                              L.list_start, L.chunk_off, L.entries, L.tile_w, 1, ks.ws);
        CV_LAUNCH_CHECK();
    }
    const int64_t wgs = queue ? L.max_items : L.max_q * ntiles;
    CV_REQUIRE(wgs < (1ll << 31), CV_EINVAL, "grid too large");
#define CV_TILES_ARGS num_rots, res, corner, d3, tab, L.ystart, L.items, L.rec, n, tiles_x, tiles_z, L.partials, L.arrivals, d_grid_obj, \
                      d_grid_rot, d_grid_scale, L.list_ctl, L.list_start, L.list_cnt, L.entries, list_mode, L.q_info, ks, L.hot, thresh, L.hot_items
#define CV_TILES_LAUNCH(MODE, WGS)                                                                           \
    do {                                                                                                      \
        if (queue) hv_fwd_tiles<true, MODE><<<dim3((unsigned)(WGS), K), TW * 64, 0, st>>>(CV_TILES_ARGS);     \
        else hv_fwd_tiles<false, MODE><<<dim3((unsigned)(WGS), K), TW * 64, 0, st>>>(CV_TILES_ARGS);          \
    } while (0)
    if (t_ev_start) CV_HIP_CHECK(hipEventRecord(t_ev_start, st));
    if (peaks) {
        CV_TILES_LAUNCH(VOTE_OBJ, wgs);
        CV_LAUNCH_CHECK();
        CV_TILES_LAUNCH(VOTE_PEAKS, std::min<int64_t>(wgs, PEAK_WGS));
    } else {
        CV_TILES_LAUNCH(VOTE_FULL, wgs);
    }
    if (t_ev_stop) CV_HIP_CHECK(hipEventRecord(t_ev_stop, st));
#undef CV_TILES_LAUNCH
#undef CV_TILES_ARGS
    CV_LAUNCH_CHECK();
    return CV_OK;
}

int cv_hv_forward_f32(const float* d_points, const float* d_xyz, const float* d_scale,
                      const float* d_obj, int64_t n, float res, int num_rots,
                      const float h_corner3[3], const int dims[3], float* d_grid_obj,
                      float* d_grid_rot, float* d_grid_scale, void* d_ws, size_t ws_bytes, int algo,
                      void* stream) {
    CV_REQUIRE(algo_ok(algo), CV_EINVAL, "algo out of range (%d: 0 auto, 1 direct, 2 tiles)", algo);
    int rc = check_common(d_points, d_xyz, d_scale, n, res, num_rots, h_corner3, dims);
    if (rc) return rc;
    CV_REQUIRE(d_obj && d_grid_obj && d_grid_rot && d_grid_scale, CV_EINVAL, "null pointer argument");
    return hv_forward_cats(d_points, d_xyz, d_scale, d_obj, n, res, num_rots, h_corner3, dims, d_grid_obj, d_grid_rot, d_grid_scale,
                           d_ws, ws_bytes, algo, 1, static_cast<hipStream_t>(stream));
}

int cv_hv_forward_cat_f32(const float* d_points, const float* d_xyz, const float* d_scale, const float* d_obj, int64_t n,
                          float res, int num_rots, const float h_corner3[3], const int dims[3], int num_cats, float* d_grid_obj,
                          float* d_grid_rot, float* d_grid_scale, void* d_ws, size_t ws_bytes, int algo, void* stream) {
    CV_REQUIRE(num_cats >= 1 && num_cats <= CV_MAX_CATEGORIES, CV_EINVAL, "num_cats out of range (%d, 1..%d)", num_cats,
               CV_MAX_CATEGORIES);
    CV_REQUIRE(algo_ok(algo), CV_EINVAL, "algo out of range (%d: 0 auto, 1 direct, 2 tiles)", algo);
    int rc = check_common(d_points, d_xyz, d_scale, n, res, num_rots, h_corner3, dims);
    if (rc) return rc;
    CV_REQUIRE(d_obj && d_grid_obj && d_grid_rot && d_grid_scale, CV_EINVAL, "null pointer argument");
    return hv_forward_cats(d_points, d_xyz, d_scale, d_obj, n, res, num_rots, h_corner3, dims, d_grid_obj, d_grid_rot, d_grid_scale,
                           d_ws, ws_bytes, algo, num_cats, static_cast<hipStream_t>(stream));
}

int cv_hv_forward_peaks_f32(const float* d_points, const float* d_xyz, const float* d_scale, const float* d_obj, int64_t n,
                            float res, int num_rots, const float h_corner3[3], const int dims[3], float* d_grid_obj,
                            float* d_grid_rot, float* d_grid_scale, void* d_ws, size_t ws_bytes, int algo, float thresh,
                            void* stream) {
    CV_REQUIRE(algo_ok(algo), CV_EINVAL, "algo out of range (%d: 0 auto, 1 direct, 2 tiles)", algo);
    CV_REQUIRE(thresh == thresh, CV_EINVAL, "thresh is not a number");
    int rc = check_common(d_points, d_xyz, d_scale, n, res, num_rots, h_corner3, dims);
    if (rc) return rc;
    CV_REQUIRE(d_obj && d_grid_obj && d_grid_rot && d_grid_scale, CV_EINVAL, "null pointer argument");
    return hv_forward_cats(d_points, d_xyz, d_scale, d_obj, n, res, num_rots, h_corner3, dims, d_grid_obj, d_grid_rot, d_grid_scale,
                           d_ws, ws_bytes, algo, 1, static_cast<hipStream_t>(stream), true, thresh);
}

int cv_hv_forward_peaks_cat_f32(const float* d_points, const float* d_xyz, const float* d_scale, const float* d_obj, int64_t n,
                                float res, int num_rots, const float h_corner3[3], const int dims[3], int num_cats,
                                float* d_grid_obj, float* d_grid_rot, float* d_grid_scale, void* d_ws, size_t ws_bytes, int algo,
                                float thresh, void* stream) {
    CV_REQUIRE(num_cats >= 1 && num_cats <= CV_MAX_CATEGORIES, CV_EINVAL, "num_cats out of range (%d, 1..%d)", num_cats,
               CV_MAX_CATEGORIES);
    CV_REQUIRE(algo_ok(algo), CV_EINVAL, "algo out of range (%d: 0 auto, 1 direct, 2 tiles)", algo);
    CV_REQUIRE(thresh == thresh, CV_EINVAL, "thresh is not a number");
    int rc = check_common(d_points, d_xyz, d_scale, n, res, num_rots, h_corner3, dims);
    if (rc) return rc;
    CV_REQUIRE(d_obj && d_grid_obj && d_grid_rot && d_grid_scale, CV_EINVAL, "null pointer argument");
    return hv_forward_cats(d_points, d_xyz, d_scale, d_obj, n, res, num_rots, h_corner3, dims, d_grid_obj, d_grid_rot, d_grid_scale,
                           d_ws, ws_bytes, algo, num_cats, static_cast<hipStream_t>(stream), true, thresh);
}

int cv_hv_backward_f32(const float* d_grad_obj, const float* d_points, const float* d_xyz,
                       const float* d_scale, const float* d_obj, int64_t n, float res, int num_rots,
                       const float h_corner3[3], const int dims[3], float* d_dxyz, float* d_dscale,
                       float* d_dobj, void* stream) {
    int rc = check_common(d_points, d_xyz, d_scale, n, res, num_rots, h_corner3, dims);
    if (rc) return rc;
    CV_REQUIRE(d_grad_obj && d_obj && d_dxyz && d_dscale && d_dobj, CV_EINVAL, "null pointer argument");
    hipStream_t st = static_cast<hipStream_t>(stream);
    const float2* tab = nullptr;
    rc = get_rot_table(num_rots, &tab);
    if (rc) return rc;
    const F3 corner{h_corner3[0], h_corner3[1], h_corner3[2]};
    const I3 d3{dims[0], dims[1], dims[2]};
    hv_bwd<<<(unsigned)((n + 3) / 4), 256, 0, st>>>(d_grad_obj, d_points, d_xyz, d_scale, d_obj, n,
                                                   num_rots, res, corner, d3, tab, d_dxyz, d_dscale,
                                                   d_dobj);
    CV_LAUNCH_CHECK();
    return CV_OK;
}

int cv_hv_count_votes_f32(const float* d_points, const float* d_xyz, const float* d_scale, int64_t n,
                          float res, int num_rots, const float h_corner3[3], const int dims[3],
                          int64_t* h_count, void* d_ws, size_t ws_bytes, void* stream) {
    int rc = check_common(d_points, d_xyz, d_scale, n, res, num_rots, h_corner3, dims);
    if (rc) return rc;
    CV_REQUIRE(h_count && d_ws && ws_bytes >= 256, CV_ENOMEM, "workspace too small");
    hipStream_t st = static_cast<hipStream_t>(stream);
    const float2* tab = nullptr;
    rc = get_rot_table(num_rots, &tab);
    if (rc) return rc;
    unsigned long long* cnt = static_cast<unsigned long long*>(d_ws);
    CV_HIP_CHECK(hipMemsetAsync(cnt, 0, sizeof(*cnt), st));
    const F3 corner{h_corner3[0], h_corner3[1], h_corner3[2]};
    const I3 d3{dims[0], dims[1], dims[2]};
    const int64_t total = n * num_rots;
    hv_count_votes<<<(unsigned)std::min<int64_t>((total + 255) / 256, 2048), 256, 0, st>>>(
        d_points, d_xyz, d_scale, n, num_rots, res, corner, d3, tab, cnt);
    CV_LAUNCH_CHECK();
    unsigned long long h = 0;
    CV_HIP_CHECK(hipMemcpyAsync(&h, cnt, sizeof h, hipMemcpyDeviceToHost, st));
    CV_HIP_CHECK(hipStreamSynchronize(st));
    *h_count = (int64_t)h;
    return CV_OK;
}

}
```

### canonicalvoting_amd/csrc/scene_exec.cpp

```cpp
#include <algorithm>
#include <atomic>
#include <chrono>
#include <cstdlib>
#include <cstring>
#include <vector>

#include "cv_common.h"

namespace {

struct Carver {
    char* base; size_t off = 0, cap;
    Carver(void* p, size_t c) : base(static_cast<char*>(p)), cap(c) {}
    template <typename T> T* take(size_t count) {
        off = cv_align_up(off, 256);
        T* r = (base && off + count * sizeof(T) <= cap) ? reinterpret_cast<T*>(base + off) : nullptr;
        off += count * sizeof(T);
        return r;
    }
};

std::atomic<int> g_scenes_inside{0};
struct SceneCount {
    int before;
// ... 81 lines not shown
        int masked[5];
        for (int i = 0; i < 5; ++i) masked[i] = off.mask_perm[i] >= 0;
        conv_ws_b = cv_sp_scene_conv_workspace_bytes(rows, masked, mask_groups, max_channels);
        return cv_sp_scene_plan_slots(&lay, &off, rows, masked_min_rows, ibuf, maps, perms);
    }
};

template <class R> int fixed_part_too_small(R* r, size_t fixed_end) {
    r->needed_ws_bytes = fixed_end * 2 + ((size_t)256 << 20);
    cv_set_error("scene workspace too small (needs at least %zu bytes)", r->needed_ws_bytes);
    return CV_ENOMEM;
}

}

extern "C" {

int cv_detect_scene_f32(const cv_scene_desc* d, cv_scene_result* r, void* stream) {
    CV_REQUIRE(d && r, CV_EINVAL, "null scene descriptor / result");
    CV_REQUIRE(d->d_coords4 && d->d_feats && d->d_points && d->n > 0 && d->ops && d->bufs && d->n_ops > 0 && d->n_bufs > 0,
               CV_EINVAL, "bad scene descriptor");
    CV_REQUIRE(d->d_out_feats && d->out_ld >= d->out_channels && d->out_channels > 0, CV_EINVAL, "bad network output buffer");
    CV_REQUIRE(d->h_pinned && d->pinned_bytes >= 256 && d->d_ws, CV_EINVAL, "pinned scratch (>= 256 bytes) and a device workspace are required");
    CV_REQUIRE(d->h_boxes && d->h_scores && d->h_classes && d->h_cand_idx && d->h_verdict && d->h_pick && d->max_candidates > 0,
               CV_EINVAL, "null result arrays");
    hipStream_t st = static_cast<hipStream_t>(stream);
    const long long n = d->n;
    std::memset(r, 0, sizeof(*r));
    CV_REQUIRE(d->conv_split_target >= 0 && d->vote_part_records >= 0, CV_EINVAL, "negative launch sizing");
    CV_REQUIRE(d->vote_algo >= 0 && d->vote_algo <= 2, CV_EINVAL, "vote_algo out of range (%d: 0 auto, 1 direct, 2 tiles)", d->vote_algo);
    SceneCount in_flight(d->adaptive_split != 0, d->conv_split_target, d->vote_part_records);
    r->scenes_in_flight = in_flight.before + 1;
    Carver cv(d->d_ws, d->ws_bytes);
    StageClock clock{d->events, st, r->host_us};
    CV_HIP_CHECK(clock.mark(0));

    SceneFront f(d);
    int32_t* h_flag = reinterpret_cast<int32_t*>(static_cast<char*>(d->h_pinned) + 64);
    const bool plan_fits = f.carve(cv);
    float* xyz = cv.take<float>((size_t)n * 3);
    float* scale = cv.take<float>((size_t)n * 3);
    float* prob = cv.take<float>((size_t)n);
    int32_t* cls = cv.take<int32_t>((size_t)n);
    int32_t* d_flag = cv.take<int32_t>(64);
    if (!plan_fits || !xyz || !scale || !prob || !cls || !d_flag) return fixed_part_too_small(r, cv.off);
    int rc = f.run(d_flag, r, clock, stream);
    if (rc != CV_OK) return rc;
    const size_t cells = f.cells;

    const size_t arena_b = cv_net_arena_bytes(d->bufs, d->n_bufs, f.rows, 5);
    const size_t vote_ws_b = cv_hv_forward_workspace_bytes(n, d->num_rots, f.dims, d->vote_algo);
    const size_t dec_ws_b = cv_decode_workspace_bytes(f.dims, n, d->max_candidates);
    char* arena = cv.take<char>(arena_b);
    char* conv_ws = cv.take<char>(f.conv_ws_b);
    char* vote_ws = cv.take<char>(std::max<size_t>(vote_ws_b, 256));
    char* dec_ws = cv.take<char>(dec_ws_b);
    float* grids = d->d_grids ? d->d_grids : cv.take<float>(6 * cells);
    r->needed_ws_bytes = cv.off + 4096;
    r->needed_grid_floats = 6 * cells;
    CV_REQUIRE(arena && conv_ws && vote_ws && dec_ws && grids, CV_ENOMEM, "scene workspace too small (needs %zu bytes)", r->needed_ws_bytes);
    CV_REQUIRE(!d->d_grids || d->grid_capacity_floats >= 6 * cells, CV_ENOMEM, "grid buffer too small (needs %zu floats)", 6 * cells);
    float* g_obj = grids;
    float* g_rot = grids + cells;
    float* g_scale = grids + 3 * cells;
    r->d_grid_obj = g_obj; r->d_grid_rot = g_rot; r->d_grid_scale = g_scale;

    const void* ext_ptr[2] = {d->d_feats, d->d_out_feats};
    const int ext_ld[2] = {d->feats_ld, d->out_ld};
    rc = cv_net_run_f32(d->ops, d->n_ops, d->bufs, d->n_bufs, f.rows, 5, arena, arena_b, ext_ptr, ext_ld, f.maps, CV_NET_MAP_SLOTS,
                        f.perms, CV_NET_PERM_SLOTS, conv_ws, f.conv_ws_b, d->use_range_flag ? d_flag : nullptr, stream);
    if (rc != CV_OK) return rc;
    clock.lap(1);
    CV_HIP_CHECK(clock.mark(1));
    rc = cv_head_joint_f32(d->d_out_feats, n, d->out_ld, d->nclasses, d->log_scale, xyz, scale, prob, cls, stream);
    if (rc != CV_OK) return rc;
    if (d->use_range_flag) CV_HIP_CHECK(hipMemcpyAsync(h_flag, d_flag, sizeof(int32_t), hipMemcpyDeviceToHost, st));
    r->d_xyz = xyz; r->d_scale = scale; r->d_prob = prob; r->d_class = cls;
    CV_HIP_CHECK(clock.mark(2));

    const float* v_xyz = d->d_xyz_in ? d->d_xyz_in : xyz;
    const float* v_scale = d->d_scale_in ? d->d_scale_in : scale;
    const float* v_prob = d->d_prob_in ? d->d_prob_in : prob;
    const int32_t* v_cls = d->d_class_in ? d->d_class_in : cls;
    rc = d->peak_quotients
             ? cv_hv_forward_peaks_f32(d->d_points, v_xyz, v_scale, v_prob, n, d->res, d->num_rots, f.mn, f.dims, g_obj, g_rot, g_scale,
                                       vote_ws, std::max<size_t>(vote_ws_b, 256), d->vote_algo, d->decode.thresh_high, stream)
             : cv_hv_forward_f32(d->d_points, v_xyz, v_scale, v_prob, n, d->res, d->num_rots, f.mn, f.dims, g_obj, g_rot, g_scale, vote_ws,
                                 std::max<size_t>(vote_ws_b, 256), d->vote_algo, stream);
    if (rc != CV_OK) return rc;
    CV_HIP_CHECK(clock.mark(3));
    clock.lap(2);
    cv_decode_params prm = d->decode;
    prm.max_iters = d->max_candidates;
    int n_cand = 0, n_boxes = 0, truncated = 0;
    const DecodeCall dc{g_obj, g_rot, g_scale, f.dims, f.mn, d->res, d->d_points, v_xyz, v_prob, v_cls, n, &prm, 0, dec_ws, dec_ws_b, &n_cand,
                        d->h_cand_idx, d->h_verdict, &n_boxes, d->h_boxes, d->h_scores, d->h_classes, &truncated, stream, d->events[4]};
    rc = cv_decode_run(dc, 1, true);
    if (rc != CV_OK) return rc;
    r->n_cand = n_cand;
    r->n_boxes = n_boxes;
    r->truncated = truncated;
    r->range_flag = d->use_range_flag ? *h_flag : 0;

    int n_det = 0;
    std::vector<float> bc, sc;
    std::vector<int32_t> idx, pick;
    for (int c = 0; c < d->nclasses; ++c) {
        bc.clear(); sc.clear(); idx.clear();
        for (int i = 0; i < n_boxes; ++i)
            if (d->h_classes[i] == c) {
                bc.insert(bc.end(), d->h_boxes + (size_t)i * 24, d->h_boxes + (size_t)i * 24 + 24);
                sc.push_back(d->h_scores[i]);
                idx.push_back(i);
            }
        if (idx.empty()) continue;
        pick.assign(idx.size(), 0);
        const int k = cv_nms_obb(bc.data(), sc.data(), (int)idx.size(), d->nms_threshold, pick.data());
        if (k < 0) return k;
        for (int j = 0; j < k; ++j) d->h_pick[n_det++] = idx[(size_t)pick[j]];
    }
    r->n_det = n_det;
    clock.lap(3);
    return CV_OK;
}

int cv_detect_scene_separate_f32(const cv_scene_separate_desc* d, cv_scene_separate_result* r, void* stream) {
    CV_REQUIRE(d && r, CV_EINVAL, "null scene descriptor / result");
    std::memset(r, 0, sizeof(*r));
    const int K = d->num_models;
    CV_REQUIRE(K >= 1 && K <= CV_MAX_CATEGORIES, CV_EINVAL, "num_models out of range (%d, 1..%d)", K, CV_MAX_CATEGORIES);
    CV_REQUIRE(d->d_coords4 && d->d_feats && d->d_points && d->n > 0 && d->ops && d->n_ops && d->bufs && d->n_bufs && d->d_out_feats,
               CV_EINVAL, "bad scene descriptor");
    for (int k = 0; k < K; ++k)
        CV_REQUIRE(d->ops[k] && d->bufs[k] && d->n_ops[k] > 0 && d->n_bufs[k] > 0 && d->d_out_feats[k], CV_EINVAL,
                   "bad program or output buffer of model %d", k);
    CV_REQUIRE(d->out_ld >= d->out_channels && d->out_channels >= 8, CV_EINVAL, "bad network output buffer");
    CV_REQUIRE(d->h_pinned && d->pinned_bytes >= 64 + 64 * (size_t)K && d->d_ws, CV_EINVAL,
               "pinned scratch (>= 64 + 64 K bytes) and a device workspace are required");
    CV_REQUIRE(d->h_boxes && d->h_scores && d->h_cand_idx && d->h_verdict && d->h_det_cat && d->h_det_box && d->max_candidates > 0,
               CV_EINVAL, "null result arrays");
    CV_REQUIRE(!!d->d_xyz_in == !!d->d_scale_in && !!d->d_xyz_in == !!d->d_prob_in, CV_EINVAL, "predictions: all three or none");
    CV_REQUIRE(d->conv_split_target >= 0 && d->vote_part_records >= 0, CV_EINVAL, "negative launch sizing");
    CV_REQUIRE(d->vote_algo >= 0 && d->vote_algo <= 2, CV_EINVAL, "vote_algo out of range (%d: 0 auto, 1 direct, 2 tiles)", d->vote_algo);
    CV_REQUIRE(d->models_per_pass >= 0, CV_EINVAL, "negative models_per_pass (%d)", d->models_per_pass);
    const int G = std::min(d->models_per_pass, K);
    if (G > 0) {
        CV_REQUIRE(d->d_model_params, CV_EINVAL, "models_per_pass needs d_model_params (cv_net_models_params_fill)");
        for (int k = 1; k < K; ++k)
            CV_REQUIRE(d->n_ops[k] == d->n_ops[0] && d->n_bufs[k] == d->n_bufs[0], CV_EINVAL,
                       "models_per_pass: the program of model %d has another length than model 0's", k);
    }
    hipStream_t st = static_cast<hipStream_t>(stream);
    const long long n = d->n;
    SceneCount in_flight(false, d->conv_split_target, d->vote_part_records);
    Carver cv(d->d_ws, d->ws_bytes);
    StageClock clock{d->events, st, r->host_us};
    CV_HIP_CHECK(clock.mark(0));

    SceneFront f(d);
    int32_t* h_flags = reinterpret_cast<int32_t*>(static_cast<char*>(d->h_pinned) + 64);
    const bool plan_fits = f.carve(cv);
    float* xyz = cv.take<float>((size_t)K * n * 3);
    float* scale = cv.take<float>((size_t)K * n * 3);
    float* prob = cv.take<float>((size_t)K * n);
    int32_t* d_flags = cv.take<int32_t>(16 * (size_t)K);
    if (!plan_fits || !xyz || !scale || !prob || !d_flags) return fixed_part_too_small(r, cv.off);
    if (d->use_range_flag) CV_HIP_CHECK(hipMemsetAsync(d_flags, 0, sizeof(int32_t) * 16 * K, st));
    int rc = f.run(nullptr, r, clock, stream);
    if (rc != CV_OK) return rc;
    const size_t cells = f.cells;

    size_t arena_b = 0;
    for (int k = 0; k < K; ++k) arena_b = std::max(arena_b, cv_net_arena_bytes(d->bufs[k], d->n_bufs[k], f.rows, 5));
    const size_t vote_ws_b = cv_hv_forward_cat_workspace_bytes(n, d->num_rots, f.dims, d->vote_algo, K);
    const size_t dec_ws_b = cv_decode_cat_workspace_bytes(f.dims, n, d->max_candidates, K);
    const size_t arena_all = G > 0 ? (size_t)G * arena_b : arena_b;
    const size_t conv_ws_all = G > 0 ? cv_net_models_workspace_bytes(f.conv_ws_b, G) : f.conv_ws_b;
    char* arena = cv.take<char>(arena_all);
    char* conv_ws = cv.take<char>(conv_ws_all);
    char* vote_ws = cv.take<char>(std::max<size_t>(vote_ws_b, 256));
    char* dec_ws = cv.take<char>(dec_ws_b);
// ... 232 lines not shown
```

### canonicalvoting_amd/pipeline.py

```python
import collections
import contextlib
import ctypes
import os

import torch

from . import _lib, decode, hv_cuda
from . import me as ME

vp = ctypes.c_void_p


class ScenePolicy(collections.namedtuple("ScenePolicy", "conv_split_target vote_part_records masked_min_rows")):
    __slots__ = ()

    def as_config(self):
        return {"conv_split_target": self.conv_split_target, "vote_part_records": self.vote_part_records,
                "masked_min_rows": self.masked_min_rows}


def policy_for_scenes_in_flight(n):
    lib_rows = ME.CoordinateManager.LIB_MASKED_MIN_ROWS
    if int(n) >= 4:
        return ScenePolicy(256, 12288, min(8192, lib_rows))
# ... 262 lines not shown
    del alive
    host["ws_hint"] = max(host["ws_hint"], int(r.needed_ws_bytes))
    if keep is not None:
        keep.update(range_flag=int(r.range_flag), needed_ws_bytes=int(r.needed_ws_bytes))
    if r.range_flag or any(r.truncated[k] for k in range(K)):
        kw = dict(decode_kw, max_candidates=M)
        if predictions is None:
            return detect_scene_separate(models, hv, coords4, feats, res, log_scale=log_scale,
                                         overlap_threshold=overlap_threshold, **kw)
        return _separate_by_calls(hv, scan_points, predictions[0], predictions[1], predictions[2], res, categories,
                                  overlap_threshold, **kw)
    return _separate_results(host, r, keep, categories, ys, n, dev, ws)


def _sep_host(dev, K, M):
    import numpy as np
    key = (dev.index, torch.cuda.current_stream(dev).cuda_stream)
    with _scene_lock:
        host = _sep_hosts.get(key)
        if host is None or host["M"] < M or host["K"] < K:
            host = _sep_hosts[key] = dict(
                M=M, K=K, ws_hint=0, pinned=torch.empty(64 + 64 * _lib.MAX_CATEGORIES, dtype=torch.uint8).pin_memory(),
                cand=np.zeros((K, M), np.int64), verdict=np.zeros((K, M), np.int32), boxes=np.zeros((K, M, 8, 3), np.float32),
                scores=np.zeros((K, M), np.float32), det_cat=np.zeros(K * M, np.int32), det_box=np.zeros(K * M, np.int32))
    return host


def _fill_separate_desc(d, host, progs, table, G, ys, decode_kw, overlap_threshold, events):
    K = len(progs)
    d.num_models = K
    if G > 0:
        d.models_per_pass, d.d_model_params = G, vp(table.data_ptr())
    ops = (vp * K)(*[ctypes.cast(p[0], vp) for p in progs])
    n_ops = (ctypes.c_int * K)(*[len(p[0]) for p in progs])
    bufs = (vp * K)(*[ctypes.cast(p[1], vp) for p in progs])
    n_bufs = (ctypes.c_int * K)(*[len(p[1]) for p in progs])
    outs = (vp * K)(*[y.data_ptr() for y in ys])
    d.ops, d.n_ops, d.bufs, d.n_bufs = ctypes.cast(ops, vp), ctypes.cast(n_ops, vp), ctypes.cast(bufs, vp), ctypes.cast(n_bufs, vp)
    d.d_out_feats, d.out_ld, d.out_channels = ctypes.cast(outs, vp), ys[0].stride(0), ys[0].shape[1]
    _fill_decode_params(d.decode, decode_kw, True)
    d.max_candidates, d.nms_threshold = host["M"], float(overlap_threshold)
    _set_events(d, events)
    d.h_pinned, d.pinned_bytes = vp(host["pinned"].data_ptr()), host["pinned"].numel()
    d.h_cand_idx, d.h_verdict = vp(host["cand"].ctypes.data), vp(host["verdict"].ctypes.data)
    d.h_boxes, d.h_scores = vp(host["boxes"].ctypes.data), vp(host["scores"].ctypes.data)
    d.h_det_cat, d.h_det_box = vp(host["det_cat"].ctypes.data), vp(host["det_box"].ctypes.data)
    return ops, n_ops, bufs, n_bufs, outs


def _separate_results(host, r, keep, categories, ys, n, dev, ws):
    K = len(categories)
    dets = [(categories[int(c)], host["boxes"][int(c), int(b)].copy(), float(host["scores"][int(c), int(b)]))
            for c, b in zip(host["det_cat"][:r.n_det], host["det_box"][:r.n_det])]
    if keep is not None:
        X, Y, Z = r.dims
        view = lambda ptr, shape: _device_view(ptr, shape, torch.float32, dev, ws)
        raw = [dict(boxes=host["boxes"][k, :r.n_boxes[k]].copy(), scores=host["scores"][k, :r.n_boxes[k]].copy(),
                    cand_idx=host["cand"][k, :r.n_cand[k]].copy(), verdict=host["verdict"][k, :r.n_cand[k]].copy())
               for k in range(K)]
        keep.update(y=ys, dims=(X, Y, Z), corner=tuple(r.corner), level_rows=list(r.level_rows), raw=raw,
                    grids=(view(r.d_grid_obj, (K, X, Y, Z)), view(r.d_grid_rot, (K, X, Y, Z, 2)),
                           view(r.d_grid_scale, (K, X, Y, Z, 3))),
                    net_pred=(view(r.d_xyz, (K, n, 3)), view(r.d_scale, (K, n, 3)), view(r.d_prob, (K, n))),
                    host_us=tuple(r.host_us))
    return dets


class _SceneHost:

    def __init__(self, max_candidates):
        import numpy as np
        self.M = max_candidates
        self.pinned = torch.empty(256, dtype=torch.uint8).pin_memory()
        self.cand = np.zeros(max_candidates, np.int64)
        self.verdict = np.zeros(max_candidates, np.int32)
        self.boxes = np.zeros((max_candidates, 8, 3), np.float32)
        self.scores = np.zeros(max_candidates, np.float32)
        self.classes = np.zeros(max_candidates, np.int32)
        self.pick = np.zeros(max_candidates, np.int32)
        self.ws_hint = 0
        self.last_host_us = (0.0, 0.0, 0.0, 0.0)


_scene_hosts = {}
_scene_lock = __import__("threading").Lock()


def detect_scene_c(model, hv, coords4, feats, res, nclasses=9, log_scale=True, scan_points=None, predictions=None,
                   max_candidates=512, keep=None, events=None, adaptive_split=False, policy=None, **decode_kw):
    import numpy as np
    L = _lib.lib()
    dev = feats.device
    n = coords4.shape[0]
    if scan_points is None:
        scan_points = (coords4[:, 1:].to(dev) * res).float().contiguous()
    pieces = 1 if ME.COMPUTE_DTYPE == "bf16" else model.PIECES
    c_ops, c_bufs, _ = model._program(dev, pieces)
    coords4 = coords4.to(device=dev, dtype=torch.int32).contiguous()
    feats = feats.contiguous()
    y = torch.empty((n, model.final.out_channels), dtype=torch.float32, device=dev)
    host = _scene_host(dev, max_candidates)
    d = _lib.SceneDesc()
    _fill_scene_desc(d, model, hv, coords4, feats, scan_points, res, policy, pieces, max(model.PLANES), log_scale)
    if predictions is not None:
        px, ps, pp, pc = predictions
        pc = pc.to(torch.int32).contiguous()
        d.d_xyz_in, d.d_scale_in, d.d_prob_in, d.d_class_in = (vp(px.data_ptr()), vp(ps.data_ptr()), vp(pp.data_ptr()),
                                                                 vp(pc.data_ptr()))
    _fill_joint_desc(d, host, c_ops, c_bufs, y, nclasses, decode_kw, adaptive_split, events)
    d.peak_quotients = 1 if keep is None else 0
    r = _lib.SceneResult()
    ws = _call_growing(L.cv_detect_scene_f32, "cv_detect_scene_f32", d, r, dev, "scene_call", host.ws_hint)
    host.ws_hint = max(host.ws_hint, int(r.needed_ws_bytes))
    host.last_host_us = tuple(r.host_us)
    if r.range_flag or r.truncated:
        if r.range_flag:
            model.range_fallbacks = getattr(model, "range_fallbacks", 0) + 1
        with torch.no_grad(), scene_policy(policy):
            x = ME.SparseTensor(feats, coords4, device=dev)
            yy = model.program_forward(x, pieces=3) if r.range_flag else x._like(y, 1)
            pred = head_joint(yy.F, nclasses, log_scale) if predictions is None else predictions
            dets, raw = decode.detect(hv, coords4[:, 1:], pred[0], pred[1], pred[2], pred[3], res, nclasses,
                                      scan_points=scan_points, **decode_kw)
        return dets, raw, yy.F
    dets, raw = _joint_results(host, r, keep, y, n, dev, ws)
    return dets, raw, y


def _scene_host(dev, max_candidates):
    key = (dev.index, torch.cuda.current_stream(dev).cuda_stream)
    with _scene_lock:
        host = _scene_hosts.get(key)
        if host is None or host.M < max_candidates:
            host = _scene_hosts[key] = _SceneHost(max_candidates)
    return host


def _fill_joint_desc(d, host, c_ops, c_bufs, y, nclasses, decode_kw, adaptive_split, events):
    d.ops, d.n_ops, d.bufs, d.n_bufs = ctypes.cast(c_ops, vp), len(c_ops), ctypes.cast(c_bufs, vp), len(c_bufs)
    d.d_out_feats, d.out_ld, d.out_channels = vp(y.data_ptr()), y.stride(0), y.shape[1]
    d.nclasses = nclasses
    _fill_decode_params(d.decode, decode_kw, False)
    d.max_candidates, d.nms_threshold = host.M, 0.3
    d.adaptive_split = 1 if adaptive_split else 0
    _set_events(d, events)
    d.h_pinned, d.pinned_bytes = vp(host.pinned.data_ptr()), host.pinned.numel()
    d.h_cand_idx, d.h_verdict = vp(host.cand.ctypes.data), vp(host.verdict.ctypes.data)
    d.h_boxes, d.h_scores, d.h_classes, d.h_pick = (vp(host.boxes.ctypes.data), vp(host.scores.ctypes.data),
                                                    vp(host.classes.ctypes.data), vp(host.pick.ctypes.data))


def _joint_results(host, r, keep, y, n, dev, ws):
    k, m = r.n_boxes, r.n_cand
    raw = dict(boxes=host.boxes[:k].copy(), scores=host.scores[:k].copy(), classes=host.classes[:k].copy(),
               cand_idx=host.cand[:m].copy(), verdict=host.verdict[:m].copy(), truncated=False)
    dets = [(int(raw["classes"][i]), raw["boxes"][i], float(raw["scores"][i])) for i in host.pick[:r.n_det]]
    if keep is not None:
        view = lambda ptr, shape, dt=torch.float32: _device_view(ptr, shape, dt, dev, ws)
        X, Y, Z = r.dims
        keep.update(y=y, dims=(X, Y, Z), corner=tuple(r.corner), level_rows=list(r.level_rows),
                    grids=(view(r.d_grid_obj, (X, Y, Z)), view(r.d_grid_rot, (X, Y, Z, 2)), view(r.d_grid_scale, (X, Y, Z, 3))),
                    net_pred=(view(r.d_xyz, (n, 3)), view(r.d_scale, (n, 3)), view(r.d_prob, (n,)),
                              view(r.d_class, (n,), torch.int32)), raw=raw)
    return dets, raw


def detect_points(model, hv, points, feats, res, predictions=None, return_inverse=False, **kw):
    coords4, index, inverse = ME.utils.quantize_device(points, res, None, return_inverse)
    gi = index.long()
    dev = coords4.device
    f = feats.to(dev)[gi]
    if predictions is not None:
        predictions = tuple(p.to(dev)[gi].contiguous() for p in predictions)
    out = detect_scene_c(model, hv, coords4, f, res, predictions=predictions, **kw)
    return out + ((index, inverse) if return_inverse else (index,))


def _points_front(front, points, feats, in_channels, recentre_from, predictions, return_inverse, with_class):
    dev = points.device
    assert points.is_cuda and points.dim() == 2 and points.shape[1] == 3, "points: a [M, 3] device tensor"
    if points.dtype not in (torch.float32, torch.float64):
        points = points.to(torch.float64)
    if points.stride(1) != 1 or points.stride(0) < 3:
        points = points.contiguous()
    m = points.shape[0]
    if m == 0:
        raise RuntimeError("sparse_quantize: empty point cloud")
    feats = feats.to(device=dev, dtype=torch.float32)
    if feats.stride(1) != 1 or feats.stride(0) < feats.shape[1]:
        feats = feats.contiguous()
    if feats.shape != (m, in_channels):
        raise ValueError("raw cloud: feats must be [%d, %d] (got %s)" % (m, in_channels, tuple(feats.shape)))
    coords4 = torch.empty((m, 4), dtype=torch.int32, device=dev)
    index = torch.empty(m, dtype=torch.int32, device=dev)
    inverse = torch.empty(m, dtype=torch.int32, device=dev) if return_inverse else None
    front.d_raw_points, front.m, front.points_ld = vp(points.data_ptr()), m, points.stride(0)
    front.points_f64 = 1 if points.dtype == torch.float64 else 0
    front.d_raw_feats, front.raw_feats_ld, front.in_channels = vp(feats.data_ptr()), feats.stride(0), in_channels
    front.recentre_from = -1 if recentre_from is None else int(recentre_from)
    front.d_coords4, front.d_index = vp(coords4.data_ptr()), vp(index.data_ptr())
    front.d_inverse = vp(inverse.data_ptr()) if return_inverse else None
    alive = [points, feats]
    if predictions is not None:
        pred = [p.to(dev).contiguous() for p in predictions]
        if with_class:
            pred[3] = pred[3].to(torch.int32).contiguous()
            front.d_raw_class = vp(pred[3].data_ptr())
        front.d_raw_xyz, front.d_raw_scale, front.d_raw_prob = vp(pred[0].data_ptr()), vp(pred[1].data_ptr()), vp(pred[2].data_ptr())
        alive += pred
    return coords4, index, inverse, alive


def _call_points(fn, name, d, r, dev, scratch_name, ws_hint):
    call = lambda _d, _r, stream: fn(ctypes.byref(d), ctypes.byref(r), stream)
    try:
        return _call_growing(call, name, d.scene, r.scene, dev, scratch_name, ws_hint)
    except _lib.CvError:
        if r.rejected:
            ME.utils.raise_rejected(r.rejected)
        raise


def detect_points_c(model, hv, points, feats, res, predictions=None, return_inverse=False, recentre_from=None, nclasses=9,
                    log_scale=True, max_candidates=512, keep=None, events=None, adaptive_split=False, policy=None, **decode_kw):
    L = _lib.lib()
    dev = points.device
    pieces = 1 if ME.COMPUTE_DTYPE == "bf16" else model.PIECES
    c_ops, c_bufs, _ = model._program(dev, pieces)
    d, r = _lib.PointsDesc(), _lib.PointsResult()
    coords4, index, inverse, alive = _points_front(d.front, points, feats, feats.shape[1], recentre_from, predictions,
                                                   return_inverse, True)
    d.front.quantization_size = float(res)
    y = torch.empty((coords4.shape[0], model.final.out_channels), dtype=torch.float32, device=dev)
    host = _scene_host(dev, max_candidates)
    _fill_scene_desc(d.scene, model, hv, None, None, None, res, policy, pieces, max(model.PLANES), log_scale)
    _fill_joint_desc(d.scene, host, c_ops, c_bufs, y, nclasses, decode_kw, adaptive_split, events)
    d.scene.peak_quotients = 1 if keep is None else 0
    ws = _call_points(L.cv_detect_points_f32, "cv_detect_points_f32", d, r, dev, "scene_call", host.ws_hint)
    del alive
    n = int(r.n)
    host.ws_hint = max(host.ws_hint, int(r.scene.needed_ws_bytes))
    host.last_host_us = tuple(r.scene.host_us)
    coords4, index, y = coords4[:n], index[:n], y[:n]
    tail = (index, inverse) if return_inverse else (index,)
    view = lambda ptr, shape, dt=torch.float32: _device_view(ptr, shape, dt, dev, ws)
    if r.scene.range_flag or r.scene.truncated:
        pred = None
        if predictions is not None:
            pred = (view(r.d_xyz_in, (n, 3)), view(r.d_scale_in, (n, 3)), view(r.d_prob_in, (n,)), view(r.d_class_in, (n,), torch.int32))
        return detect_scene_c(model, hv, coords4, view(r.d_feats, (n, d.front.in_channels)), res, nclasses=nclasses,
                              log_scale=log_scale, predictions=pred, max_candidates=max_candidates, keep=keep, events=events,
                              adaptive_split=adaptive_split, policy=policy, **decode_kw) + tail
    if keep is not None:
        keep.update(scan_points=view(r.d_points, (n, 3)), feats=view(r.d_feats, (n, d.front.in_channels)),
                    host_us=tuple(r.scene.host_us), host_us_front=float(r.host_us_front), front_ws_bytes=int(r.front_ws_bytes))
    dets, raw = _joint_results(host, r.scene, keep, y, n, dev, ws)
    return (dets, raw, y) + tail


def detect_points_separate_c(models, hv, points, feats, res, predictions=None, models_per_pass=None, return_inverse=False,
                             recentre_from=None, policy=None, keep=None, events=None, log_scale=True, overlap_threshold=0.3,
                             max_candidates=512, **decode_kw):
    import numpy as np
    decode_kw.setdefault("separate_variant", True)
    decode_kw.setdefault("err_thresh", float(np.float32(0.3)))
    L = _lib.lib()
    dev = points.device
    categories = list(models.keys())
    mods = [models[c] for c in categories]
    K = len(mods)
    if not 1 <= K <= _lib.MAX_CATEGORIES:
        raise ValueError("detect_points_separate_c: 1..%d models (got %d)" % (_lib.MAX_CATEGORIES, K))
    pieces = 1 if ME.COMPUTE_DTYPE == "bf16" else mods[0].PIECES
    G = int(models_per_pass or 0)
    if G < 0:
        raise ValueError("detect_points_separate_c: models_per_pass must be >= 0 (got %d)" % G)
    if G > 0:
        progs, table = model_params_table(mods, dev, pieces)
    else:
        progs, table = [m._program(dev, pieces) for m in mods], None
    d, r = _lib.PointsSeparateDesc(), _lib.PointsSeparateResult()
    coords4, index, inverse, alive = _points_front(d.front, points, feats, feats.shape[1], recentre_from, predictions,
                                                   return_inverse, False)
    d.front.quantization_size = float(res)
    m = coords4.shape[0]
    ys = [torch.empty((m, mod.final.out_channels), dtype=torch.float32, device=dev) for mod in mods]
    M = int(max_candidates)
    host = _sep_host(dev, K, M)
    _fill_scene_desc(d.scene, mods[0], hv, None, None, None, res, policy, pieces, max(max(mod.PLANES) for mod in mods), log_scale)
    alive.append(_fill_separate_desc(d.scene, host, progs, table, G, ys, decode_kw, overlap_threshold, events))
    ws = _call_points(L.cv_detect_points_separate_f32, "cv_detect_points_separate_f32", d, r, dev, "scene_call_separate",
                      host["ws_hint"])
    del alive
    n = int(r.n)
    host["ws_hint"] = max(host["ws_hint"], int(r.scene.needed_ws_bytes))
    coords4, index, ys = coords4[:n], index[:n], [y[:n] for y in ys]
    tail = (index, inverse) if return_inverse else (index,)
    if keep is not None:
        keep.update(range_flag=int(r.scene.range_flag), needed_ws_bytes=int(r.scene.needed_ws_bytes), coords4=coords4)
    if r.scene.range_flag or any(r.scene.truncated[k] for k in range(K)):
        view = lambda ptr, shape: _device_view(ptr, shape, torch.float32, dev, ws)
        pred = None
        if predictions is not None:
            pred = (view(r.d_xyz_in, (K, n, 3)), view(r.d_scale_in, (K, n, 3)), view(r.d_prob_in, (K, n)))
        return (detect_scene_separate_c(models, hv, coords4, view(r.d_feats, (n, d.front.in_channels)), res, predictions=pred,
                                        policy=policy, keep=keep, events=events, log_scale=log_scale,
                                        overlap_threshold=overlap_threshold, max_candidates=M, models_per_pass=models_per_pass,
                                        **decode_kw),) + tail
    return (_separate_results(host, r.scene, keep, categories, ys, n, dev, ws),) + tail


def last_scene_host_us(dev=None):
    dev = torch.device("cuda", torch.cuda.current_device()) if dev is None else dev
    host = _scene_hosts.get((dev.index, torch.cuda.current_stream(dev).cuda_stream))
    return host.last_host_us if host is not None else None


def _device_view(ptr, shape, dtype, dev, owner):
    import numpy as np
    count = int(np.prod(shape))
# ... 5 lines not shown
```

### include/cv_hip.h

```cpp
#ifndef CV_HIP_H
#define CV_HIP_H

#include <stddef.h>
#include <stdint.h>

#ifdef __cplusplus
extern "C" {
#endif

#define CV_OK 0
#define CV_EINVAL (-22)
#define CV_ENOMEM (-12)
#define CV_EHIP (-5)
#define CV_ERANGE (-34)

#define CV_ABI_VERSION 6
int cv_abi_version(void);
const char* cv_last_error(void);


size_t cv_hv_minmax_workspace_bytes(void);
int cv_hv_minmax_f32(const float* d_points, int64_t n, float* h_min3, float* h_max3,
                     void* d_ws, size_t ws_bytes, void* stream);
int cv_hv_minmax_async_f32(const float* d_points, int64_t n, float* h_minmax6, void* d_ws, size_t ws_bytes,
                           void* stream);

int cv_hv_grid_dims_f32(const float h_min3[3], const float h_max3[3], float res, int dims_out[3]);

size_t cv_hv_forward_workspace_bytes(int64_t n, int num_rots, const int dims[3], int algo);

int cv_hv_forward_f32(const float* d_points, const float* d_xyz, const float* d_scale,
                      const float* d_obj, int64_t n, float res, int num_rots,
                      const float h_corner3[3], const int dims[3], float* d_grid_obj,
                      float* d_grid_rot, float* d_grid_scale, void* d_ws, size_t ws_bytes,
                      int algo, void* stream);

#define CV_MAX_CATEGORIES 16
size_t cv_hv_forward_cat_workspace_bytes(int64_t n, int num_rots, const int dims[3], int algo, int num_cats);
int cv_hv_forward_cat_f32(const float* d_points, const float* d_xyz, const float* d_scale, const float* d_obj, int64_t n,
                          float res, int num_rots, const float h_corner3[3], const int dims[3], int num_cats, float* d_grid_obj,
                          float* d_grid_rot, float* d_grid_scale, void* d_ws, size_t ws_bytes, int algo, void* stream);

int cv_hv_forward_peaks_f32(const float* d_points, const float* d_xyz, const float* d_scale, const float* d_obj, int64_t n,
                            float res, int num_rots, const float h_corner3[3], const int dims[3], float* d_grid_obj,
                            float* d_grid_rot, float* d_grid_scale, void* d_ws, size_t ws_bytes, int algo, float thresh,
                            void* stream);
int cv_hv_forward_peaks_cat_f32(const float* d_points, const float* d_xyz, const float* d_scale, const float* d_obj, int64_t n,
                                float res, int num_rots, const float h_corner3[3], const int dims[3], int num_cats,
                                float* d_grid_obj, float* d_grid_rot, float* d_grid_scale, void* d_ws, size_t ws_bytes, int algo,
                                float thresh, void* stream);

int cv_hv_set_part_records(int records);
int cv_hv_set_part_records_thread(int records);
int cv_hv_set_kernel_events(void* ev_start, void* ev_stop);

int cv_hv_backward_f32(const float* d_grad_obj, const float* d_points, const float* d_xyz,
                       const float* d_scale, const float* d_obj, int64_t n, float res,
                       int num_rots, const float h_corner3[3], const int dims[3], float* d_dxyz,
                       float* d_dscale, float* d_dobj, void* stream);

int cv_hv_count_votes_f32(const float* d_points, const float* d_xyz, const float* d_scale, int64_t n,
                          float res, int num_rots, const float h_corner3[3], const int dims[3],
                          int64_t* h_count, void* d_ws, size_t ws_bytes, void* stream);

typedef struct cv_decode_params {
    float thresh_high;
    float thresh_low;
    float valid_ratio;
    int elimination;
    float prob_thresh;
    int elim_hi_plus1;
    int max_iters;
    double err_thresh;
} cv_decode_params;

size_t cv_decode_workspace_bytes(const int dims[3], int64_t n, int max_iters);

int cv_decode_f32(float* d_grid_obj, const float* d_grid_rot, const float* d_grid_scale,
                  const int dims[3], const float h_corner3[3], float res, const float* d_points,
                  const float* d_xyz, const float* d_prob, const int32_t* d_class, int64_t n,
                  const cv_decode_params* params, int mutate_grid, void* d_ws, size_t ws_bytes,
                  int* h_n_cand, int64_t* h_cand_idx, int32_t* h_verdict, int* h_n_boxes,
                  float* h_boxes, float* h_scores, int32_t* h_classes, int* h_truncated, void* stream);

size_t cv_decode_cat_workspace_bytes(const int dims[3], int64_t n, int max_iters, int num_cats);
int cv_decode_cat_f32(float* d_grid_obj, const float* d_grid_rot, const float* d_grid_scale, const int dims[3],
                      const float h_corner3[3], float res, const float* d_points, const float* d_xyz, const float* d_prob,
                      const int32_t* d_class, int64_t n, int num_cats, const cv_decode_params* params, int mutate_grid, void* d_ws,
                      size_t ws_bytes, int* h_n_cand, int64_t* h_cand_idx, int32_t* h_verdict, int* h_n_boxes, float* h_boxes,
                      float* h_scores, int32_t* h_classes, int* h_truncated, void* stream);

double cv_iou_obb(const float* h_box1, const float* h_box2);
int cv_nms_obb(const float* h_boxes, const float* h_scores, int n, double thr, int32_t* h_pick);


long long cv_sp_table_capacity(long long n);
size_t cv_sp_levels_workspace_bytes(long long n);

int cv_sp_build_levels(int32_t* const* d_coords, unsigned long long* const* d_keys,
                       int32_t* const* d_vals, long long n, long long cap, int num_levels,
                       int32_t* d_counts, int32_t* h_counts, void* d_ws, size_t ws_bytes, void* stream);

#define CV_QUANTIZE_MAX_CLOUDS 256
size_t cv_sp_quantize_workspace_bytes(long long m);
int cv_sp_quantize_f32(const float* d_points, long long m, long long ld, float quantization_size, int floor_only,
                       const long long* h_offsets, int n_clouds, int32_t* d_coords4, int32_t* d_index, int32_t* d_inverse,
                       int32_t* d_counts, int32_t* h_counts, void* d_ws, size_t ws_bytes, void* stream);
int cv_sp_quantize_f64(const double* d_points, long long m, long long ld, double quantization_size, int floor_only,
                       const long long* h_offsets, int n_clouds, int32_t* d_coords4, int32_t* d_index, int32_t* d_inverse,
                       int32_t* d_counts, int32_t* h_counts, void* d_ws, size_t ws_bytes, void* stream);

#define CV_GATHER_MAX_JOBS 8
typedef struct cv_gather_job {
    const void* d_src; long long src_ld;
    void* d_dst; long long dst_ld;
    int width;
    int recentre_from;
} cv_gather_job;
int cv_sp_voxel_rows_f32(const int32_t* d_coords4, const int32_t* d_index, long long n, float res, float* d_points_out,
                         const cv_gather_job* jobs, int n_jobs, void* stream);

typedef struct cv_scan_rows_desc {
    const int32_t* d_coords4; const int32_t* d_index; long long n;
    long long m_points;
    const float* d_points; long long points_ld;
    const uint8_t* d_rgb;
    const int32_t* d_owner;
    const double* d_minv; const float* d_model_scale; const int32_t* d_model_cls; int n_models;
    const double* d_colour; const double* d_jitter; int n_clouds;
    int use_xyz, recentre;
    float* d_feats; long long feats_ld;
    float* d_xyz; long long xyz_ld;
    float* d_scale; long long scale_ld;
// ... 387 lines not shown
```

Measured before the change: 676.3.

## Emit decode candidate list directly from the peaks vote kernel

```diff
diff --git a/canonicalvoting_amd/_lib.py b/canonicalvoting_amd/_lib.py
--- a/canonicalvoting_amd/_lib.py
+++ b/canonicalvoting_amd/_lib.py
@@ -222,6 +222,10 @@
     "cv_hv_forward_peaks_f32": (ctypes.c_int, [vp, vp, vp, vp, ctypes.c_int64, ctypes.c_float, ctypes.c_int,
                                                c_float_p, c_int_p, vp, vp, vp, vp, ctypes.c_size_t,
                                                ctypes.c_int, ctypes.c_float, vp]),
+    "cv_hv_forward_list_f32": (ctypes.c_int, [vp, vp, vp, vp, ctypes.c_int64, ctypes.c_float, ctypes.c_int,
+                                              c_float_p, c_int_p, vp, vp, vp, vp, ctypes.c_size_t,
+                                              ctypes.c_int, ctypes.c_float, ctypes.c_int, vp, ctypes.c_size_t, c_int_p, vp]),
+    "cv_decode_list_layout": (ctypes.c_int, [c_int_p, ctypes.c_int, ctypes.POINTER(ctypes.c_size_t)]),
     "cv_hv_forward_peaks_cat_f32": (ctypes.c_int, [vp, vp, vp, vp, ctypes.c_int64, ctypes.c_float, ctypes.c_int, c_float_p, c_int_p,
                                                    ctypes.c_int, vp, vp, vp, vp, ctypes.c_size_t, ctypes.c_int, ctypes.c_float,
                                                    vp]),
diff --git a/canonicalvoting_amd/csrc/cv_common.h b/canonicalvoting_amd/csrc/cv_common.h
--- a/canonicalvoting_amd/csrc/cv_common.h
+++ b/canonicalvoting_amd/csrc/cv_common.h
@@ -81,8 +81,46 @@
     int* h_n_cand; int64_t* h_cand_idx; int32_t* h_verdict; int* h_n_boxes; float* h_boxes; float* h_scores; int32_t* h_classes;
     int* h_truncated;
     void* stream; void* ev_done;
+    int list_ready;
 };
 int cv_decode_run(const DecodeCall& c, int num_cats, bool need_class);
+
+constexpr int CV_DEC_CTR_WORDS = 16;
+struct CvDecodeList {
+    float* val;
+    unsigned* xy;
+    int* z;
+    float* geo;
+    int64_t cap;
+    unsigned* list_n;
+};
+int cv_decode_list_view(const int dims[3], int max_iters, void* d_ws, size_t ws_bytes, CvDecodeList* out);
+__device__ __forceinline__ void cv_decode_list_entry(const CvDecodeList& L, unsigned p, float v, int x, int y, int z, float r0,
+                                                     float r1, float s0, float s1, float s2) {
+    L.val[p] = v;
+    L.xy[p] = (unsigned)x | ((unsigned)y << 16);
+    L.z[p] = z;
+    const float rot = (float)atan2((double)r1, (double)r0);
+    L.geo[0 * L.cap + p] = (float)cos((double)rot);
+    L.geo[1 * L.cap + p] = (float)sin((double)rot);
+    L.geo[2 * L.cap + p] = s0;
+    L.geo[3 * L.cap + p] = s1;
+    L.geo[4 * L.cap + p] = s2;
+}
+__device__ __forceinline__ unsigned cv_decode_list_reserve(const CvDecodeList& L, bool hit) {
+    const uint64_t m = __ballot(hit);
+    if (m == 0) return 0u;
+    const int lane = (int)(threadIdx.x & 63u);
+    const int leader = __ffsll((unsigned long long)m) - 1;
+    unsigned pos = 0;
+    if (lane == leader) pos = atomicAdd(L.list_n, (unsigned)__popcll(m));
+    pos = __shfl(pos, leader);
+    return pos + (unsigned)__builtin_amdgcn_mbcnt_hi((uint32_t)(m >> 32), __builtin_amdgcn_mbcnt_lo((uint32_t)m, 0));
+}
+int cv_hv_forward_list(const float* d_points, const float* d_xyz, const float* d_scale, const float* d_obj, int64_t n, float res,
+                       int num_rots, const float h_corner3[3], const int dims[3], float* d_grid_obj, float* d_grid_rot,
+                       float* d_grid_scale, void* d_ws, size_t ws_bytes, int algo, float thresh, const CvDecodeList& dl,
+                       int* list_ready, void* stream);
 int cv_sp_sort_rows_ex(const int32_t* d_coords, long long n, int32_t* d_sorted, int32_t* d_perm, int32_t* d_inv, void* d_ws,
                        size_t ws_bytes, bool single_batch, void* stream, bool bounds_prefilled);
 int cv_sp_scene_plan_ex(const int32_t* d_input, long long n, int32_t* d_perm, int32_t* d_inv, int32_t* const* d_coords,
diff --git a/canonicalvoting_amd/csrc/hv_decode.hip b/canonicalvoting_amd/csrc/hv_decode.hip
--- a/canonicalvoting_amd/csrc/hv_decode.hip
+++ b/canonicalvoting_amd/csrc/hv_decode.hip
@@ -44,7 +44,7 @@
     return ((int)(xy & 0xffffu) * geo.Y + (int)(xy >> 16)) * geo.Z + z;
 }
 
-constexpr int CTR_WORDS = 16;
+constexpr int CTR_WORDS = CV_DEC_CTR_WORDS;
 constexpr int CTR_LIST_N = 0;
 constexpr int CTR_N_CAND = 4;
 
@@ -71,11 +71,6 @@
 
 __device__ __forceinline__ void lds_barrier() {
     asm volatile("s_waitcnt lgkmcnt(0)\n\ts_barrier" ::: "memory");
-}
-
-__device__ __forceinline__ int lanes_below(uint64_t mask) {
-    return __builtin_amdgcn_mbcnt_hi((uint32_t)(mask >> 32),
-                                     __builtin_amdgcn_mbcnt_lo((uint32_t)mask, 0));
 }
 
 __global__ __launch_bounds__(256) void dec_compact(const float* __restrict__ g_obj,
@@ -92,25 +87,13 @@
         float v = 0.f;
         bool hit = false;
         if (i < G) { v = g_obj[i]; hit = v >= thresh; }
-        const uint64_t m = __ballot(hit);
-        if (m == 0) continue;
-        unsigned pos = 0;
-        const int lane = threadIdx.x & 63;
-        const int leader = __ffsll((unsigned long long)m) - 1;
-        if (lane == leader) pos = atomicAdd(list_n, (unsigned)__popcll(m));
-        pos = __shfl(pos, leader);
+        const CvDecodeList V{L.val, L.xy, L.z, L.geo, L.cap, list_n};
+        const unsigned p = cv_decode_list_reserve(V, hit);
         if (hit) {
-            const unsigned p = pos + lanes_below(m);
             const int id = (int)i;
-            L.val[p] = v;
             const int z = id % geo.Z, y = (id / geo.Z) % geo.Y, x = id / (geo.Z * geo.Y);
-            L.xy[p] = (unsigned)x | ((unsigned)y << 16);
-            L.z[p] = z;
-            const float r0 = g_rot[(int64_t)id * 2], r1 = g_rot[(int64_t)id * 2 + 1];
-            const float rot = (float)atan2((double)r1, (double)r0);
-            L.geo[0 * L.cap + p] = (float)cos((double)rot);
-            L.geo[1 * L.cap + p] = (float)sin((double)rot);
-            for (int k = 0; k < 3; ++k) L.geo[(2 + k) * L.cap + p] = g_scale[(int64_t)id * 3 + k];
+            cv_decode_list_entry(V, p, v, x, y, z, g_rot[(int64_t)id * 2], g_rot[(int64_t)id * 2 + 1], g_scale[(int64_t)id * 3],
+                                 g_scale[(int64_t)id * 3 + 1], g_scale[(int64_t)id * 3 + 2]);
         }
     }
 }
@@ -749,7 +732,9 @@
 
 int cv_decode_run(const DecodeCall& c, int K, bool need_class) {
     CV_REQUIRE(K >= 1 && K <= CV_MAX_CATEGORIES, CV_EINVAL, "num_cats out of range (%d, 1..%d)", K, CV_MAX_CATEGORIES);
-    CV_REQUIRE(c.d_grid_obj && c.d_grid_rot && c.d_grid_scale && c.dims && c.h_corner3 && c.d_points && c.d_xyz && c.d_prob &&
+    const bool list_ready = c.list_ready != 0;
+    CV_REQUIRE(!list_ready || (K == 1 && !c.mutate_grid), CV_EINVAL, "a list made by the vote: one category, no grid to mutate");
+    CV_REQUIRE((list_ready || (c.d_grid_obj && c.d_grid_rot && c.d_grid_scale)) && c.dims && c.h_corner3 && c.d_points && c.d_xyz && c.d_prob &&
                    (c.d_class || !need_class) && c.params && c.d_ws && c.h_n_cand && c.h_cand_idx && c.h_verdict && c.h_n_boxes &&
                    c.h_boxes && c.h_scores && c.h_classes,
                CV_EINVAL, "null pointer argument");
@@ -777,15 +762,17 @@
     CV_REQUIRE(host != nullptr, CV_ENOMEM, "pinned host buffer of %zu bytes", (size_t)K * RL.total);
     const CatStride ks{K > 1 ? (int64_t)W.total : 0, n, G};
 
-    if (K == 1) CV_HIP_CHECK(hipMemsetAsync(w.counters, 0, sizeof(unsigned) * CTR_WORDS, st));
-    else {
-        dec_zero_counters<<<dim3(1, K), 64, 0, st>>>(w, ks.ws);
+    Geo geo{dims[0], dims[1], dims[2], {c.h_corner3[0], c.h_corner3[1], c.h_corner3[2]}, c.res};
+    if (!list_ready) {
+        if (K == 1) CV_HIP_CHECK(hipMemsetAsync(w.counters, 0, sizeof(unsigned) * CTR_WORDS, st));
+        else {
+            dec_zero_counters<<<dim3(1, K), 64, 0, st>>>(w, ks.ws);
+            CV_LAUNCH_CHECK();
+        }
+        const int cblocks = (int)std::min<int64_t>((G + 255) / 256, 2048);
+        dec_compact<<<dim3(cblocks, K), 256, 0, st>>>(c.d_grid_obj, c.d_grid_rot, c.d_grid_scale, geo, G, params->thresh_high, w, ks);
         CV_LAUNCH_CHECK();
     }
-    Geo geo{dims[0], dims[1], dims[2], {c.h_corner3[0], c.h_corner3[1], c.h_corner3[2]}, c.res};
-    const int cblocks = (int)std::min<int64_t>((G + 255) / 256, 2048);
-    dec_compact<<<dim3(cblocks, K), 256, 0, st>>>(c.d_grid_obj, c.d_grid_rot, c.d_grid_scale, geo, G, params->thresh_high, w, ks);
-    CV_LAUNCH_CHECK();
     static const long long big_cells = getenv("CV_DEC_BIG_CELLS") ? atoll(getenv("CV_DEC_BIG_CELLS")) : (4ll << 20);
     if (G > big_cells) dec_greedy_dispatch_big<<<dim3(1, K), GREEDY_T_BIG, 0, st>>>(geo, *params, w, ks.ws);
     else dec_greedy_dispatch<<<dim3(1, K), GREEDY_T, 0, st>>>(geo, *params, w, ks.ws);
@@ -818,12 +805,34 @@
     return CV_OK;
 }
 
+int cv_decode_list_view(const int dims[3], int max_iters, void* d_ws, size_t ws_bytes, CvDecodeList* out) {
+    CV_REQUIRE(dims && d_ws && out, CV_EINVAL, "null pointer argument");
+    CV_REQUIRE(dims[0] > 0 && dims[1] > 0 && dims[2] > 0 && dims[0] < 65536 && dims[1] < 65536 && dims[2] < 65536, CV_EINVAL,
+               "bad grid dims");
+    const int64_t G = (int64_t)dims[0] * dims[1] * dims[2];
+    CV_REQUIRE(G < (1ll << 31), CV_EINVAL, "grid too large");
+    CV_REQUIRE(max_iters > 0 && max_iters <= 65536, CV_EINVAL, "max_iters out of range");
+    const WsLayout W(G, max_iters);
+    CV_REQUIRE(ws_bytes >= W.total, CV_ENOMEM, "workspace too small (%zu < %zu)", ws_bytes, W.total);
+    const Ws w = W.at(static_cast<char*>(d_ws));
+    *out = CvDecodeList{w.L.val, w.L.xy, w.L.z, w.L.geo, w.L.cap, w.list_n()};
+    return CV_OK;
+}
+
 extern "C" {
 
 size_t cv_decode_workspace_bytes(const int dims[3], int64_t n, int max_iters) {
     if (!dims || max_iters <= 0) return 0;
     (void)n;
     return WsLayout((int64_t)dims[0] * dims[1] * dims[2], max_iters).total;
+}
+
+int cv_decode_list_layout(const int dims[3], int max_iters, size_t out6[6]) {
+    CV_REQUIRE(dims && out6 && max_iters > 0 && dims[0] > 0 && dims[1] > 0 && dims[2] > 0, CV_EINVAL, "bad argument");
+    const WsLayout W((int64_t)dims[0] * dims[1] * dims[2], max_iters);
+    out6[0] = W.off_val; out6[1] = W.off_xy; out6[2] = W.off_z; out6[3] = W.off_geo; out6[4] = W.off_counters;
+    out6[5] = (size_t)W.cells;
+    return CV_OK;
 }
 
 size_t cv_decode_cat_workspace_bytes(const int dims[3], int64_t n, int max_iters, int num_cats) {
diff --git a/canonicalvoting_amd/csrc/hv_vote.hip b/canonicalvoting_amd/csrc/hv_vote.hip
--- a/canonicalvoting_amd/csrc/hv_vote.hip
+++ b/canonicalvoting_amd/csrc/hv_vote.hip
@@ -238,7 +238,7 @@
                                                     int* __restrict__ cursor,
                                                     int* __restrict__ part_start, int4* __restrict__ q_info, int max_q,
                                                     int* __restrict__ chunk_start, int* __restrict__ bin_of_chunk,
-                                                    int part_records, int64_t ks_ws) {
+                                                    int part_records, int64_t ks_ws, unsigned* __restrict__ dec_counters) {
     ycount = cat_ws(ycount, ks_ws); ystart = cat_ws(ystart, ks_ws); cursor = cat_ws(cursor, ks_ws);
     part_start = cat_ws(part_start, ks_ws); q_info = cat_ws(q_info, ks_ws);
     chunk_start = cat_ws(chunk_start, ks_ws); bin_of_chunk = cat_ws(bin_of_chunk, ks_ws);
@@ -266,6 +266,8 @@
                                              for (int p2 = 0; p2 < v; ++p2) bin_of_chunk[excl + p2] = i;
                                          });
         if (lane == 0) chunk_start[Y] = total;
+    } else if (dec_counters && lane < CV_DEC_CTR_WORDS) {
+        dec_counters[lane] = 0u;
     }
 }
 
@@ -660,8 +662,9 @@
     int* __restrict__ arrivals, float* __restrict__ g_obj, float* __restrict__ g_rot,
     float* __restrict__ g_scale, const int* __restrict__ list_ctl, const int* __restrict__ list_start, const int* __restrict__ list_cnt,
     const int2* __restrict__ entries, int list_mode ,
-    int4* __restrict__ hot, float thresh, int4* __restrict__ hot_items, const float2* __restrict__ tab) {
+    int4* __restrict__ hot, float thresh, int4* __restrict__ hot_items, const CvDecodeList& dl, const float2* __restrict__ tab) {
     constexpr int NCH = vote_channels(MODE);
+    const bool list_out = MODE != VOTE_FULL && dl.val != nullptr;
     __shared__ TileSharedT<MODE> sh;
     __shared__ int last_flag;
     __shared__ int hot_lds[MODE == VOTE_OBJ ? 4 : 1];
@@ -681,8 +684,8 @@
             const int lx = i / TZ, lz = i % TZ;
             if (lx < nx0 && lz < nz0) {
                 const int64_t cell = ((int64_t)(x0 + lx) * Y + y) * Z + z0 + lz;
-                if (MODE != VOTE_PEAKS) g_obj[cell] = 0.f;
-                if (MODE != VOTE_OBJ) {
+                if (MODE != VOTE_PEAKS && !list_out) g_obj[cell] = 0.f;
+                if (MODE != VOTE_OBJ && !list_out) {
                     reinterpret_cast<float2*>(g_rot)[cell] = make_float2(0.f, 0.f);
                     g_scale[cell * 3 + 0] = 0.f; g_scale[cell * 3 + 1] = 0.f; g_scale[cell * 3 + 2] = 0.f;
                 }
@@ -1000,7 +1003,7 @@
             const int lx = i / TZ, lz = i % TZ;
             if (lx < nx && lz < nz) {
                 const float v = (float)fx_value(sh.acc[acc_idx(0, i)]);
-                g_obj[((int64_t)(x0 + lx) * Y + y) * Z + z0 + lz] = v;
+                if (!list_out) g_obj[((int64_t)(x0 + lx) * Y + y) * Z + z0 + lz] = v;
                 if (v >= thresh) {
                     atomicMin(&hot_lds[0], lx); atomicMax(&hot_lds[1], lx);
                     atomicMin(&hot_lds[2], lz); atomicMax(&hot_lds[3], lz);
@@ -1008,6 +1011,12 @@
             }
         }
         __syncthreads();
+        if (list_out && hot_lds[0] <= hot_lds[1]) {
+            for (int i = threadIdx.x; i < TCELLS; i += TW * 64) {
+                const int lx = i / TZ, lz = i % TZ;
+                if (lx < nx && lz < nz) g_obj[((int64_t)(x0 + lx) * Y + y) * Z + z0 + lz] = (float)fx_value(sh.acc[acc_idx(0, i)]);
+            }
+        }
         if (threadIdx.x == 0) {
             hot[y * ntiles + tile] = make_int4(hot_lds[0], hot_lds[1], hot_lds[2], hot_lds[3]);
             if (hot_lds[0] <= hot_lds[1]) {
@@ -1016,17 +1025,26 @@
             }
         }
     } else if constexpr (MODE == VOTE_PEAKS) {
+        static_assert(TCELLS % (TW * 64) == 0, "every lane of a wave takes the same number of cells: the list append is a ballot");
         for (int i = threadIdx.x; i < TCELLS; i += TW * 64) {
             const int lx = i / TZ, lz = i % TZ;
-            if (lx < box.x0 || lx > box.x1 || lz < box.z0 || lz > box.z1) continue;
+            const bool in_box = lx >= box.x0 && lx <= box.x1 && lz >= box.z0 && lz <= box.z1;
             const int64_t cell = ((int64_t)(x0 + lx) * Y + y) * Z + z0 + lz;
-            const float v = g_obj[cell];
-            if (!(v >= thresh)) continue;
-            const double d = (double)v + 1e-7;
-#pragma unroll
-            for (int j = 0; j < 2; ++j) g_rot[cell * 2 + j] = (float)((double)(float)fx_value(sh.acc[acc_idx(j, i)]) / d);
-#pragma unroll
-            for (int j = 0; j < 3; ++j) g_scale[cell * 3 + j] = (float)((double)(float)fx_value(sh.acc[acc_idx(2 + j, i)]) / d);
+            const float v = in_box ? g_obj[cell] : 0.f;
+            const bool hit = in_box && v >= thresh;
+            float q[5] = {0.f, 0.f, 0.f, 0.f, 0.f};
+            if (hit) {
+                const double d = (double)v + 1e-7;
+#pragma unroll
+                for (int j = 0; j < 5; ++j) q[j] = (float)((double)(float)fx_value(sh.acc[acc_idx(j, i)]) / d);
+            }
+            if (list_out) {
+                const unsigned p = cv_decode_list_reserve(dl, hit);
+                if (hit && (int64_t)p < dl.cap) cv_decode_list_entry(dl, p, v, x0 + lx, y, z0 + lz, q[0], q[1], q[2], q[3], q[4]);
+            } else if (hit) {
+                g_rot[cell * 2 + 0] = q[0]; g_rot[cell * 2 + 1] = q[1];
+                g_scale[cell * 3 + 0] = q[2]; g_scale[cell * 3 + 1] = q[3]; g_scale[cell * 3 + 2] = q[4];
+            }
         }
     } else {
         for (int i = threadIdx.x; i < TCELLS; i += TW * 64) {
@@ -1063,7 +1081,8 @@
     int* __restrict__ arrivals, float* __restrict__ g_obj, float* __restrict__ g_rot,
     float* __restrict__ g_scale, const int* __restrict__ list_ctl, const int* __restrict__ list_start, const int* __restrict__ list_cnt,
     const int2* __restrict__ entries, int list_mode ,
-    const int4* __restrict__ q_info, CatStride ks, int4* __restrict__ hot, float thresh, int4* __restrict__ hot_items) {
+    const int4* __restrict__ q_info, CatStride ks, int4* __restrict__ hot, float thresh, int4* __restrict__ hot_items,
+    CvDecodeList dl) {
     ystart = cat_ws(ystart, ks.ws); items = cat_ws(items, ks.ws); rec = cat_ws(rec, ks.ws);
     partials = cat_ws(partials, ks.ws); arrivals = cat_ws(arrivals, ks.ws); list_ctl = cat_ws(list_ctl, ks.ws);
     list_start = cat_ws(list_start, ks.ws); list_cnt = cat_ws(list_cnt, ks.ws); entries = cat_ws(entries, ks.ws);
@@ -1072,7 +1091,7 @@
     if (MODE != VOTE_FULL) { hot = cat_ws(hot, ks.ws); hot_items = cat_ws(hot_items, ks.ws); }
     const int ntiles = tiles_x * tiles_z;
 #define CV_TILE_ITEM_ARGS R, res, corner, dims, ystart, rec, rec_stride, tiles_x, tiles_z, partials, arrivals, g_obj, g_rot, g_scale, \
-                          list_ctl, list_start, list_cnt, entries, list_mode, hot, thresh, hot_items
+                          list_ctl, list_start, list_cnt, entries, list_mode, hot, thresh, hot_items, dl
     if (MODE == VOTE_PEAKS) {
         const int count = arrivals[dims.y * ntiles];
         if ((int)blockIdx.x >= count) return;
@@ -1391,8 +1410,9 @@
 static int hv_forward_cats(const float* d_points, const float* d_xyz, const float* d_scale, const float* d_obj, int64_t n,
                            float res, int num_rots, const float h_corner3[3], const int dims[3], float* d_grid_obj,
                            float* d_grid_rot, float* d_grid_scale, void* d_ws, size_t ws_bytes, int algo, int K,
-                           hipStream_t st, bool peaks = false, float thresh = 0.f) {
+                           hipStream_t st, bool peaks = false, float thresh = 0.f, const CvDecodeList* list = nullptr) {
     int rc = CV_OK;
+    const CvDecodeList dl = list ? *list : CvDecodeList{};
     const float2* tab = nullptr;
     rc = get_rot_table(num_rots, &tab);
     if (rc) return rc;
@@ -1438,7 +1458,7 @@
     hv_prep_scan<<<dim3(1, K), 256, 0, st>>>(L.ycount, Y, L.ystart, L.cursor, L.part_start, L.q_info, (int)L.max_q, L.chunk_start,
                                              L.bin_of_chunk,
                                              (int)(t_part_records > 0 ? t_part_records : g_part_records.load(std::memory_order_relaxed)),
-                                             ks.ws);
+                                             ks.ws, dl.val ? dl.list_n : nullptr);
     CV_LAUNCH_CHECK();
     hv_prep_scatter<<<dim3(prep_wgs, K), PREP_THREADS, 0, st>>>(d_points, d_xyz, d_scale, d_obj, L.fy, n, Y, res, corner, L.cursor,
                                                                  L.rec, n, ks);
@@ -1461,7 +1481,7 @@
     const int64_t wgs = queue ? L.max_items : L.max_q * ntiles;
     CV_REQUIRE(wgs < (1ll << 31), CV_EINVAL, "grid too large");
 #define CV_TILES_ARGS num_rots, res, corner, d3, tab, L.ystart, L.items, L.rec, n, tiles_x, tiles_z, L.partials, L.arrivals, d_grid_obj, \
-                      d_grid_rot, d_grid_scale, L.list_ctl, L.list_start, L.list_cnt, L.entries, list_mode, L.q_info, ks, L.hot, thresh, L.hot_items
+                      d_grid_rot, d_grid_scale, L.list_ctl, L.list_start, L.list_cnt, L.entries, list_mode, L.q_info, ks, L.hot, thresh, L.hot_items, dl
 #define CV_TILES_LAUNCH(MODE, WGS)                                                                           \
     do {                                                                                                      \
         if (queue) hv_fwd_tiles<true, MODE><<<dim3((unsigned)(WGS), K), TW * 64, 0, st>>>(CV_TILES_ARGS);     \
@@ -1534,6 +1554,40 @@
     CV_REQUIRE(d_obj && d_grid_obj && d_grid_rot && d_grid_scale, CV_EINVAL, "null pointer argument");
     return hv_forward_cats(d_points, d_xyz, d_scale, d_obj, n, res, num_rots, h_corner3, dims, d_grid_obj, d_grid_rot, d_grid_scale,
                            d_ws, ws_bytes, algo, num_cats, static_cast<hipStream_t>(stream), true, thresh);
+}
+
+}
+
+int cv_hv_forward_list(const float* d_points, const float* d_xyz, const float* d_scale, const float* d_obj, int64_t n, float res,
+                       int num_rots, const float h_corner3[3], const int dims[3], float* d_grid_obj, float* d_grid_rot,
+                       float* d_grid_scale, void* d_ws, size_t ws_bytes, int algo, float thresh, const CvDecodeList& dl,
+                       int* list_ready, void* stream) {
+    CV_REQUIRE(list_ready, CV_EINVAL, "null pointer argument");
+    *list_ready = 0;
+    CV_REQUIRE(algo_ok(algo), CV_EINVAL, "algo out of range (%d: 0 auto, 1 direct, 2 tiles)", algo);
+    CV_REQUIRE(thresh == thresh, CV_EINVAL, "thresh is not a number");
+    int rc = check_common(d_points, d_xyz, d_scale, n, res, num_rots, h_corner3, dims);
+    if (rc) return rc;
+    const bool list = pick_algo(algo, n, num_rots) == 2 && thresh > 0.f && dl.val && dl.xy && dl.z && dl.geo && dl.list_n &&
+                      dl.cap >= (int64_t)dims[0] * dims[1] * dims[2];
+    CV_REQUIRE(d_obj && d_grid_obj && (list || (d_grid_rot && d_grid_scale)), CV_EINVAL, "null pointer argument");
+    rc = hv_forward_cats(d_points, d_xyz, d_scale, d_obj, n, res, num_rots, h_corner3, dims, d_grid_obj, d_grid_rot, d_grid_scale, d_ws,
+                         ws_bytes, algo, 1, static_cast<hipStream_t>(stream), true, thresh, list ? &dl : nullptr);
+    if (rc == CV_OK && list) *list_ready = 1;
+    return rc;
+}
+
+extern "C" {
+
+int cv_hv_forward_list_f32(const float* d_points, const float* d_xyz, const float* d_scale, const float* d_obj, int64_t n, float res,
+                           int num_rots, const float h_corner3[3], const int dims[3], float* d_grid_obj, float* d_grid_rot,
+                           float* d_grid_scale, void* d_ws, size_t ws_bytes, int algo, float thresh, int max_iters, void* d_decode_ws,
+                           size_t decode_ws_bytes, int* list_ready, void* stream) {
+    CvDecodeList dl{};
+    const int rc = cv_decode_list_view(dims, max_iters, d_decode_ws, decode_ws_bytes, &dl);
+    if (rc) return rc;
+    return cv_hv_forward_list(d_points, d_xyz, d_scale, d_obj, n, res, num_rots, h_corner3, dims, d_grid_obj, d_grid_rot, d_grid_scale,
+                              d_ws, ws_bytes, algo, thresh, dl, list_ready, stream);
 }
 
 int cv_hv_backward_f32(const float* d_grad_obj, const float* d_points, const float* d_xyz,
diff --git a/canonicalvoting_amd/csrc/scene_exec.cpp b/canonicalvoting_amd/csrc/scene_exec.cpp
--- a/canonicalvoting_amd/csrc/scene_exec.cpp
+++ b/canonicalvoting_amd/csrc/scene_exec.cpp
@@ -187,7 +187,16 @@
     const float* v_scale = d->d_scale_in ? d->d_scale_in : scale;
     const float* v_prob = d->d_prob_in ? d->d_prob_in : prob;
     const int32_t* v_cls = d->d_class_in ? d->d_class_in : cls;
-    rc = d->peak_quotients
+    int list_ready = 0;
+    CvDecodeList dl{};
+    if (d->peak_quotients == 2) {
+        rc = cv_decode_list_view(f.dims, d->max_candidates, dec_ws, dec_ws_b, &dl);
+        if (rc != CV_OK) return rc;
+    }
+    rc = d->peak_quotients == 2
+             ? cv_hv_forward_list(d->d_points, v_xyz, v_scale, v_prob, n, d->res, d->num_rots, f.mn, f.dims, g_obj, g_rot, g_scale, vote_ws,
+                                  std::max<size_t>(vote_ws_b, 256), d->vote_algo, d->decode.thresh_high, dl, &list_ready, stream)
+         : d->peak_quotients
              ? cv_hv_forward_peaks_f32(d->d_points, v_xyz, v_scale, v_prob, n, d->res, d->num_rots, f.mn, f.dims, g_obj, g_rot, g_scale,
                                        vote_ws, std::max<size_t>(vote_ws_b, 256), d->vote_algo, d->decode.thresh_high, stream)
              : cv_hv_forward_f32(d->d_points, v_xyz, v_scale, v_prob, n, d->res, d->num_rots, f.mn, f.dims, g_obj, g_rot, g_scale, vote_ws,
@@ -199,9 +208,11 @@
     prm.max_iters = d->max_candidates;
     int n_cand = 0, n_boxes = 0, truncated = 0;
     const DecodeCall dc{g_obj, g_rot, g_scale, f.dims, f.mn, d->res, d->d_points, v_xyz, v_prob, v_cls, n, &prm, 0, dec_ws, dec_ws_b, &n_cand,
-                        d->h_cand_idx, d->h_verdict, &n_boxes, d->h_boxes, d->h_scores, d->h_classes, &truncated, stream, d->events[4]};
+                        d->h_cand_idx, d->h_verdict, &n_boxes, d->h_boxes, d->h_scores, d->h_classes, &truncated, stream, d->events[4],
+                        list_ready};
     rc = cv_decode_run(dc, 1, true);
     if (rc != CV_OK) return rc;
+    if (list_ready) { r->d_grid_obj = nullptr; r->d_grid_rot = nullptr; r->d_grid_scale = nullptr; }
     r->n_cand = n_cand;
     r->n_boxes = n_boxes;
     r->truncated = truncated;
diff --git a/canonicalvoting_amd/pipeline.py b/canonicalvoting_amd/pipeline.py
--- a/canonicalvoting_amd/pipeline.py
+++ b/canonicalvoting_amd/pipeline.py
@@ -368,6 +368,8 @@
         self.last_host_us = (0.0, 0.0, 0.0, 0.0)
 
 
+PEAKS_WITHOUT_KEEP = 2
+
 _scene_hosts = {}
 _scene_lock = __import__("threading").Lock()
 
@@ -394,7 +396,7 @@
         d.d_xyz_in, d.d_scale_in, d.d_prob_in, d.d_class_in = (vp(px.data_ptr()), vp(ps.data_ptr()), vp(pp.data_ptr()),
                                                                  vp(pc.data_ptr()))
     _fill_joint_desc(d, host, c_ops, c_bufs, y, nclasses, decode_kw, adaptive_split, events)
-    d.peak_quotients = 1 if keep is None else 0
+    d.peak_quotients = PEAKS_WITHOUT_KEEP if keep is None else 0
     r = _lib.SceneResult()
     ws = _call_growing(L.cv_detect_scene_f32, "cv_detect_scene_f32", d, r, dev, "scene_call", host.ws_hint)
     host.ws_hint = max(host.ws_hint, int(r.needed_ws_bytes))
@@ -521,7 +523,7 @@
     host = _scene_host(dev, max_candidates)
     _fill_scene_desc(d.scene, model, hv, None, None, None, res, policy, pieces, max(model.PLANES), log_scale)
     _fill_joint_desc(d.scene, host, c_ops, c_bufs, y, nclasses, decode_kw, adaptive_split, events)
-    d.scene.peak_quotients = 1 if keep is None else 0
+    d.scene.peak_quotients = PEAKS_WITHOUT_KEEP if keep is None else 0
     ws = _call_points(L.cv_detect_points_f32, "cv_detect_points_f32", d, r, dev, "scene_call", host.ws_hint)
     del alive
     n = int(r.n)
diff --git a/include/cv_hip.h b/include/cv_hip.h
--- a/include/cv_hip.h
+++ b/include/cv_hip.h
@@ -49,6 +49,11 @@
                                 float res, int num_rots, const float h_corner3[3], const int dims[3], int num_cats,
                                 float* d_grid_obj, float* d_grid_rot, float* d_grid_scale, void* d_ws, size_t ws_bytes, int algo,
                                 float thresh, void* stream);
+int cv_hv_forward_list_f32(const float* d_points, const float* d_xyz, const float* d_scale, const float* d_obj, int64_t n, float res,
+                           int num_rots, const float h_corner3[3], const int dims[3], float* d_grid_obj, float* d_grid_rot,
+                           float* d_grid_scale, void* d_ws, size_t ws_bytes, int algo, float thresh, int max_iters, void* d_decode_ws,
+                           size_t decode_ws_bytes, int* list_ready, void* stream);
+int cv_decode_list_layout(const int dims[3], int max_iters, size_t out6[6]);
 
 int cv_hv_set_part_records(int records);
 int cv_hv_set_part_records_thread(int records);
diff --git a/profiles/launch_table.py b/profiles/launch_table.py
--- /dev/null
+++ b/profiles/launch_table.py
@@ -0,0 +1,57 @@
+import collections
+import csv
+import json
+import statistics
+import os
+import sys
+
+sys.path.insert(0, os.path.dirname(os.path.abspath(__file__)))
+
+from in_flight_summary import family, find
+
+
+def main():
+    tdir, bench_json, label = sys.argv[1:4]
+    bench = json.loads(open(bench_json).read().strip().splitlines()[-1])
+    steps = bench["steps"]
+    tfile = find(tdir, "kernel_trace.csv")
+    rows = list(csv.DictReader(open(tfile)))
+
+    def grid(r):
+        g = [int(r[k]) for k in ("Grid_Size_X", "Grid_Size_Y", "Grid_Size_Z")]
+        w = [max(1, int(r[k])) for k in ("Workgroup_Size_X", "Workgroup_Size_Y", "Workgroup_Size_Z")]
+        return g[0] // w[0], max(1, g[1] // w[1])
+
+    ev = sorted((int(r["Start_Timestamp"]), int(r["End_Timestamp"]), r["Kernel_Name"], grid(r)) for r in rows)
+    heads = [e for e in ev if family(e[2]) == "head"]
+    iso = 2 * 4 + max(min(steps, 48), 24)
+    assert len(heads) >= steps + iso, (len(heads), steps, iso)
+    t_lo, t_hi = heads[-(steps + iso) + 20][0], heads[-(iso + 20) - 1][1]
+    t_iso = heads[-(iso - 8) - 1][1]
+    dur = {"in flight": collections.defaultdict(list), "alone": collections.defaultdict(list)}
+    for s, e, n, g in ev:
+        short = n.replace("(anonymous namespace)::", "").replace("void ", "").split("(")[0]
+        where = "in flight" if t_lo < s < t_hi else "alone" if s > t_iso else None
+        if where:
+            dur[where][short].append((e - s) * 1e-3)
+    scenes = {"in flight": len([h for h in heads if t_lo < h[1] <= t_hi]), "alone": iso - 8}
+    print("%s: %.1f scenes/s under the tracer; %d scenes in flight, %d alone" % (label, bench["value"], scenes["in flight"], scenes["alone"]))
+    print("%-60s %22s %22s" % ("kernel", "in flight us (per scene)", "alone us (per scene)"))
+    tot = {"in flight": 0.0, "alone": 0.0}
+    cnt = {"in flight": 0.0, "alone": 0.0}
+    for k in sorted(set(dur["in flight"]) | set(dur["alone"])):
+        cells = []
+        for w in ("in flight", "alone"):
+            v = dur[w].get(k)
+            if v:
+                tot[w] += sum(v) / scenes[w]
+                cnt[w] += len(v) / scenes[w]
+                cells.append("%10.1f (%6.2f)" % (statistics.median(v), len(v) / scenes[w]))
+            else:
+                cells.append("%19s" % "-")
+        print("%-60s %22s %22s" % (k[:60], cells[0], cells[1]))
+    print("%-60s %22.2f %22.2f   launches per scene" % ("all", cnt["in flight"], cnt["alone"]))
+    print("%-60s %22.1f %22.1f   sum of kernel durations per scene, us" % ("all", tot["in flight"], tot["alone"]))
+
+
+main()
```

After: 675.0. Within noise of the previous version (-0.2%).
